# mp3guy/ElasticFusion

Measured on AMD Instinct MI355X. Metric: frames/s per GPU, 640x480 3-level ICP+fuse, higher is better.
Workload: dtype f32

## Files before the change

elasticfusion_amd/build.py:

```python
from __future__ import annotations

import os
import subprocess
import sys

HERE = os.path.dirname(os.path.abspath(__file__))
CSRC = os.path.join(HERE, "csrc")
LIB = os.path.join(HERE, "libefusion_hip.so")
FAST_LIB = os.path.join(HERE, "libefusion_hip_fast.so")
NOFMA_LIB = LIB
VARIANTS = {
    "fast": ["-DEF_FAST_BUILD"],
    "reforder": ["-DEF_FAST_BUILD", "-DEF_REF_ORDER"],
    "nofma_fast": ["-DEF_FORCE_FAST_ORDER"],
    "clocks": ["-DEF_STAGE_CLOCKS"],
    "fast_clocks": ["-DEF_FAST_BUILD", "-DEF_STAGE_CLOCKS"],
    "ldlt_wave": ["-DEF_LDLT_WAVE"],
    "ldlt_wave_clocks": ["-DEF_LDLT_WAVE", "-DEF_STAGE_CLOCKS"],
    "nopairs": ["-DEF_NO_VISIT_PAIRS"],
    "nopairs_clocks": ["-DEF_NO_VISIT_PAIRS", "-DEF_STAGE_CLOCKS"],
    "p_icp": ["-DEF_RT_WITH_PAIRS_ICP"],
    "p_search": ["-DEF_RT_WITH_PAIRS_SEARCH"],
    "p_rgb": ["-DEF_RT_WITH_PAIRS_RGB"],
    "p_all": ["-DEF_RT_WITH_PAIRS_ICP", "-DEF_RT_WITH_PAIRS_SEARCH", "-DEF_RT_WITH_PAIRS_RGB"],
    "shfl": ["-DEF_RT_SHFL_REDUCE"],
    "sepsc": ["-DEF_SEPARATE_SIN_COS"],
    "pyrstages": ["-DEF_PYR_STAGES"],
    "deep": ["-DEF_DEEP_PIPE"],
    "sepinputs": ["-DEF_SEPARATE_INPUTS"],
    "sepmerge": ["-DEF_SEPARATE_MERGE"],
    "pre_vpair": ["-DEF_PRE_VPAIR"],
    "prep_late": ["-DEF_RT_PREPARE_LATE"],
    "p_nostream": ["-DEF_RT_NO_PAIRS_STREAM"],
    "sepscan": ["-DEF_SEPARATE_SCAN"],
    "endwave": ["-DEF_END_ONE_WAVE"],
    "pre_pertap": ["-DEF_PRE_SCALE_PER_TAP"],
    "assoc_late": ["-DEF_ASSOC_LATE_LOADS"],
    "resolveall": ["-DEF_RESOLVE_ALL_MAPS"],
    "splat_early": ["-DEF_SPLAT_EARLY_LOADS"],
    "resolvetally": ["-DEF_RESOLVE_TALLY"],
    "modeone": ["-DEF_FT_MODE_ONE"],
    "modeone_clocks": ["-DEF_FT_MODE_ONE", "-DEF_STAGE_CLOCKS"],
    "norepl": ["-DEF_FT_REPL=1", "-DEF_FT_REPL_A=1"],
    "norepl_clocks": ["-DEF_FT_REPL=1", "-DEF_FT_REPL_A=1", "-DEF_STAGE_CLOCKS"],
    "lanesweep": ["-DEF_FT_LANE_SWEEP"],
    "lanesweep_clocks": ["-DEF_FT_LANE_SWEEP", "-DEF_STAGE_CLOCKS"],
    "pipepoll": ["-DEF_FT_PIPELINED_POLL"],
    "pipepoll_clocks": ["-DEF_FT_PIPELINED_POLL", "-DEF_STAGE_CLOCKS"],
    "alltaps": ["-DEF_CLEAN_ALL_TAPS"],
    "r6m": ["-DEF_SEPARATE_SCAN", "-DEF_END_ONE_WAVE"],
}
SHIM_LIB = os.path.join(HERE, "libefusion.so")
SOURCES = ["ef_track_kernels.hip", "ef_map_kernels.hip", "ef_context.hip", "ef_ferns.hip"]
FLAGS = ["--offload-arch=gfx950", "-O3", "-std=c++17", "-fPIC", "-ffp-contract=off", "-fno-fast-math",
         "-Wall", "-Wno-unused-function", "-Wno-unused-result"]


def _hipcc() -> str:
    for c in (os.environ.get("HIPCC"), "/opt/rocm/bin/hipcc", "hipcc"):
        if c and (os.path.isabs(c) and os.path.exists(c) or not os.path.isabs(c)):
            return c
    raise RuntimeError("hipcc not found")


def needs_build() -> bool:
    if not os.path.exists(LIB) or not os.path.exists(SHIM_LIB):
        return True
    t = os.path.getmtime(LIB)
    root = os.path.dirname(HERE)
    deps = [os.path.join(CSRC, f) for f in os.listdir(CSRC) if f.endswith((".hip", ".inc", ".hpp", ".h"))]
    deps += [os.path.join(root, "include", "ef_hip.h"), os.path.join(root, "include", "ElasticFusion.h"), os.path.join(root, "include", "efusion_klg.hpp"), os.path.join(root, "include", "efusion_jpeg.hpp"),
             os.path.join(root, "tools", "efusion_replay.cpp"), __file__]
    replay = os.path.join(HERE, "efusion_replay")
    return not os.path.exists(replay) or any(os.path.getmtime(d) > min(t, os.path.getmtime(replay)) for d in deps)


def build(force: bool = False, verbose: bool = False) -> str:
    if not force and not needs_build():
        return LIB
    objs = []
    procs = []
    for src in SOURCES:
        obj = os.path.join(CSRC, src.replace(".hip", ".o"))
        cmd = [_hipcc(), *FLAGS, *os.environ.get("EF_HIPCC_FLAGS", "").split(), "-c", os.path.join(CSRC, src), "-o", obj]
        if verbose:
            print(" ".join(cmd), flush=True)
        procs.append((src, subprocess.Popen(cmd, stdout=subprocess.PIPE, stderr=subprocess.STDOUT, text=True)))
        objs.append(obj)
    for src, p in procs:
        out, _ = p.communicate()
        if p.returncode != 0:
            raise RuntimeError(f"hipcc failed on {src}:\n{out}")
        if verbose and out.strip():
            print(out)
    cmd = [_hipcc(), "--offload-arch=gfx950", "-shared", "-fPIC", "-o", LIB, *objs, "-Wl,-rpath,/opt/rocm/lib"]
    r = subprocess.run(cmd, stdout=subprocess.PIPE, stderr=subprocess.STDOUT, text=True)
    if r.returncode != 0:
        raise RuntimeError(f"link failed:\n{r.stdout}")
    cmd = [_hipcc(), "--offload-arch=gfx950", "-O2", "-std=c++17", "-fPIC", "-ffp-contract=off", "-shared", "-o", SHIM_LIB,
           os.path.join(CSRC, "efusion_shim.hip"), "-L" + HERE, "-lefusion_hip", "-lz", "-ldl", "-Wl,-rpath,$ORIGIN", "-Wl,-rpath,/opt/rocm/lib"]
    r = subprocess.run(cmd, stdout=subprocess.PIPE, stderr=subprocess.STDOUT, text=True)
    if r.returncode != 0:
        raise RuntimeError(f"libefusion.so build failed:\n{r.stdout}")
    replay = os.path.join(HERE, "efusion_replay")
    cmd = ["g++", "-O2", "-std=c++17", os.path.join(os.path.dirname(HERE), "tools", "efusion_replay.cpp"), "-o", replay, "-L" + HERE,
           "-lefusion", "-lefusion_hip", "-lz", "-ldl", "-Wl,-rpath,$ORIGIN", "-Wl,-rpath,/opt/rocm/lib", "-Wl,-rpath-link," + HERE]
    r = subprocess.run(cmd, stdout=subprocess.PIPE, stderr=subprocess.STDOUT, text=True)
    if r.returncode != 0:
        raise RuntimeError(f"efusion_replay build failed:\n{r.stdout}")
    return LIB


def build_variant(name: str, extra_flags: list[str]) -> str:
    extra_flags = VARIANTS.get(name, []) + list(extra_flags)
    target = os.path.join(HERE, f"libefusion_hip_{name}.so")
    objs = []
    procs = []
    for src in SOURCES:
        obj = os.path.join(CSRC, src.replace(".hip", f"_{name}.o"))
        procs.append((src, subprocess.Popen([_hipcc(), *FLAGS, *extra_flags, "-c", os.path.join(CSRC, src), "-o", obj], stdout=subprocess.PIPE,
                                            stderr=subprocess.STDOUT, text=True)))
        objs.append(obj)
    for src, p in procs:
        out, _ = p.communicate()
        if p.returncode != 0:
            raise RuntimeError(f"hipcc failed on {src}:\n{out}")
    r = subprocess.run([_hipcc(), "--offload-arch=gfx950", "-shared", "-fPIC", "-o", target, *objs, "-Wl,-rpath,/opt/rocm/lib"], stdout=subprocess.PIPE,
                       stderr=subprocess.STDOUT, text=True)
    if r.returncode != 0:
        raise RuntimeError(f"link failed:\n{r.stdout}")
    return target


if __name__ == "__main__":
    if "--variant" in sys.argv:
        i = sys.argv.index("--variant")
        print(build_variant(sys.argv[i + 1], sys.argv[i + 2:]))
    else:
        print(build(force="--force" in sys.argv, verbose=True))
```

elasticfusion_amd/csrc/ef_context.hip:

```cpp
#include <hip/hip_runtime.h>
#include <math.h>
#include <cmath>
#include <stdio.h>
#include <string.h>
#include <limits>
#include <string>
#include <thread>
#include <vector>

#include "../../include/ef_hip.h"
#include "ef_linalg_dev.hpp"
#include "ef_solve_dev.hpp"
#include "ef_map.hpp"
#include "ef_deform_solver.hpp"
#include "ef_track.hpp"

namespace {

thread_local std::string g_create_error;

struct StageTimer {
  const char* name;
  hipEvent_t a, b;
  bool used;
};

}

struct ef_ctx {
  ef_config cfg;
  hipStream_t stream = nullptr;
  bool own_stream = false;
  std::string err;
  efm::Cam cam;
  eft::Intr intr;
  const float maxDepthProcessed = 20.0f;
  uint8_t* rgb = nullptr;
  uint16_t* depth_raw = nullptr;
  uint16_t* depth_filtered = nullptr;
  float* depth_metric = nullptr;
  float* depth_metric_filtered = nullptr;
  uint8_t* rgb_alt = nullptr;
  uint16_t* depth_raw_alt = nullptr;
  uint16_t* depth_filtered_alt = nullptr;
  float* depth_metric_alt = nullptr;
  float* depth_metric_filtered_alt = nullptr;
  hipStream_t in_stream = nullptr;
  hipEvent_t ev_input_done = nullptr, ev_track_done = nullptr, ev_staged = nullptr;
  hipEvent_t ev_frame_done[2] = {nullptr, nullptr};
  int frame_parity = 0;
  int overlap_mode = 1;
  bool overlap = false;
  bool events_live = false;
  static constexpr int RING = 3;
  uint8_t* h_rgb_ring[RING] = {};
  uint16_t* h_depth_ring[RING] = {};
  uint8_t* d_rgb_ring[RING] = {};
  uint16_t* d_depth_ring[RING] = {};
  hipEvent_t ev_h2d[RING] = {};
  hipStream_t copy_stream = nullptr;
  unsigned host_seq = 0;
  unsigned mark_value = 0;
  unsigned* h_consumed = nullptr;
  unsigned* d_consumed = nullptr;
  unsigned* h_abort = nullptr;
  unsigned* d_abort = nullptr;
  eft::Pyramid pyr{};
  eft::TrackState* st = nullptr;
  efm::IndexMaps im{};
  efm::PredictMaps pm{};
  efm::FillMaps fm{};
  unsigned long long* zbuf = nullptr;
  efm::SurfelSoA maps[2]{};
  int cur = 0;
  efm::SurfelSoA shadow{};
  bool reference_download = false;
  uint32_t capacity = 0;
  uint32_t* winner = nullptr;
  efm::Candidates cand{};
  efm::CompactScratch cs{};
  int* overflow = nullptr;
  double* traj = nullptr;
  int traj_cap = 0;
  std::vector<int64_t> stamps;
  int tick = 1;
  std::vector<void*> allocs;
  bool tally_by_consumer = false;
  bool tally_pending = false;
  bool timing = false;
  std::vector<StageTimer> timers;
  float* graph_dev = nullptr;
  int graph_nodes = 0, graph_is_fern = 0;
  float* synth_depth = nullptr;
  float* rays = nullptr;
  int icp_count_thresh = 35000;
  float icp_err_thresh = 5e-05f, cov_thresh = 1e-05f;
  int deforms = 0;
  const float* bil_table = nullptr;
  eft::Pyramid pyr2{};
  eft::TrackState* st2 = nullptr;
  efm::PredictMaps old{};
  float* cons_dev = nullptr;
  float* h_cons = nullptr;
  eft::TrackState* h_states = nullptr;
  ef_loop_solver solver = nullptr;
  void* solver_user = nullptr;
  bool builtin_solver = false;
  int64_t last_deform_time = 0;
  float* nodes_dev = nullptr;
  std::vector<float> h_nodes;
  ef_local_loop loop{};
  std::vector<double> loop_constraints;
  std::vector<float> loop_graph;
  ef_closure* closure = nullptr;
  ef_global_loop gloop{};
  std::string fern_tracker_error;
  int fern_w = 0, fern_h = 0;
  uchar4* view_img_dev = nullptr;
  float4* view_vert_dev = nullptr;
  float4* view_norm_dev = nullptr;
  uint8_t* h_view = nullptr;
  eft::Pyramid pyr3{};
  eft::TrackState* st3 = nullptr;
  eft::Intr intr3{};
  float4* fern_maps_dev = nullptr;
  float* h_nodes_pinned = nullptr;
  int* fern_table_dev = nullptr;
  int fern_num = 0, fern_table_version = -1;
  uint8_t* fern_codes_dev = nullptr;
  uint8_t* h_codes = nullptr;
  uint8_t* h_codes_end = nullptr;
  uint8_t* h_view_end = nullptr;
  hipEvent_t ev_end_record = nullptr;
  bool end_pending = false, end_lost = false;
  int end_tick = 0;
  int n_nodes_host = 0;
  double h_pose[16] = {1, 0, 0, 0, 0, 1, 0, 0, 0, 0, 1, 0, 0, 0, 0, 1};
  bool reloc = false, lost = false, last_frame_recovery = false, tracking_ok = true;
  int tracking_count = 0;
  eft::TrackState h_reloc{};
  bool use_graph = false;
  bool track_only = false;
  bool no_resident = false;
  bool fused_step = false;
  int persistent = 1;
  struct TrackGraph { hipGraphExec_t exec = nullptr; const void* key = nullptr; eft::TrackParams tp{}; eft::TrackTail tail{}; };
  TrackGraph tgraph[2];
  int ktime_every = 0;
  std::vector<hipEvent_t> kt_start, kt_stop;
  eft::KernelProbe probe{nullptr, nullptr, 0, 0};
  std::vector<hipEvent_t> ks_start, ks_stop;
  eft::KernelProbe probe_splat{nullptr, nullptr, 0, 0};
  std::vector<hipEvent_t> ka_start, ka_stop;
  eft::KernelProbe probe_all{nullptr, nullptr, 0, 0};
  hipStream_t debug_stream = nullptr;
  unsigned long long* render_zbuf = nullptr;
  size_t render_zbuf_n = 0;
  uint8_t* render_out = nullptr;
  size_t render_out_bytes = 0;
  bool ids_on = false, ids_bad = false;
  unsigned* ids_state = nullptr;
  int label_C = 0, label_cur = 0;
  float* label_tab[2] = {};
  uint32_t* label_ids[2] = {};
  size_t label_rows = 0, label_bound = 0;
  size_t label_known = 0, label_known_frames = 0, label_ev_frames = 0;
  unsigned* label_count_h = nullptr;
  hipEvent_t label_ev = nullptr;
  bool label_ev_pending = false;
  uint32_t* label_index = nullptr;
  size_t label_index_n = 0;
  uint8_t* label_stage = nullptr;
  size_t label_stage_bytes = 0;
  uint64_t map_gen = 1, query_gen = 0;
  float query_cell = EF_QUERY_DEFAULT_CELL, query_built_cell = 0.f;
  int query_lanes = 0;
  float4* query_sorted = nullptr;
  uint32_t* query_rows = nullptr;
  size_t query_cap = 0;
  uint32_t* query_cells = nullptr;
  size_t query_cells_cap = 0;
  uint32_t query_nb = 0, query_n = 0;
  uint8_t* query_stage = nullptr;
  size_t query_stage_bytes = 0;
  uint8_t* reg_slabs = nullptr;
  size_t reg_slabs_bytes = 0;
  double* reg_sums_h = nullptr;
  uint8_t* reg_stage = nullptr;
  size_t reg_stage_bytes = 0;
};

namespace {

#define EF_HIP(ctx, expr)                                                                       \
  do {                                                                                          \
    hipError_t _e = (expr);                                                                     \
    if (_e != hipSuccess) {                                                                     \
      (ctx)->err = std::string(#expr) + ": " + hipGetErrorString(_e);                           \
      return EF_EHIP;                                                                           \
    }                                                                                           \
  } while (0)

struct DeviceGuard {
  int prev = -1;
  bool switched = false;
  explicit DeviceGuard(const ef_ctx* c) {
    if (c && hipGetDevice(&prev) == hipSuccess && prev != c->cfg.device) switched = hipSetDevice(c->cfg.device) == hipSuccess;
  }
  ~DeviceGuard() {
    if (switched) (void)hipSetDevice(prev);
  }
  DeviceGuard(const DeviceGuard&) = delete;
  DeviceGuard& operator=(const DeviceGuard&) = delete;
};

template <typename T>
int dev_alloc(ef_ctx* c, T** p, size_t n, int fill = 0) {
  void* q = nullptr;
  hipError_t e = hipMalloc(&q, n * sizeof(T));
  if (e != hipSuccess) {
    c->err = std::string("hipMalloc: ") + hipGetErrorString(e);
    return EF_ENOMEM;
  }
  e = hipMemsetAsync(q, fill, n * sizeof(T), c->stream);
  if (e != hipSuccess) {
// ... 459 lines not shown
  const uint8_t* rgb_in = fold_copies ? rgb_src : c->rgb;
#ifdef EF_SEPARATE_INPUTS
  const bool joint_inputs = false;
#else
  const bool joint_inputs = track_this && !overlap && !c->timing;
#endif
  if (!joint_inputs && !efm::preprocess_depth(depth_in, W, H, c->cfg.depth_cut, c->depth_filtered, c->depth_metric, c->depth_metric_filtered, sb, 0u,
                             track_this ? rgb_in : nullptr, c->pyr.nextImage[0], fold_copies ? c->rgb : nullptr, c->bil_table)) {
    c->err = "bilateral weight table missing on this device";
    return EF_EHIP;
  }
  timer_end(c, "Preprocess");
  if (overlap && overlap_mode == 2) EF_HIP(c, hipStreamWaitEvent(sb, c->ev_track_done, 0));
  if (track_this && overlap)
    eft::build_pyramids_frame_side(c->pyr, c->depth_filtered, c->intr, c->maxDepthProcessed, nullptr, sb, nullptr);
  if (overlap) EF_HIP(c, hipEventRecord(c->ev_input_done, sb));

  const bool rgbOnly = c->cfg.rgb_only != 0;
  if ((int)c->stamps.size() >= c->traj_cap) {
    const int r = grow_trajectory(c);
    if (r != EF_OK) return r;
  }
  const int log_slot = (int)c->stamps.size();
  c->stamps.push_back(timestamp);
  if (c->tick == 1) {
    if (overlap) EF_HIP(c, hipStreamWaitEvent(s, c->ev_input_done, 0));
    timer_begin(c, "feedbackBuffers");
    efm::seed_map(c->cam, c->rgb, c->depth_metric, c->depth_metric_filtered, c->tick, c->maxDepthProcessed, c->maps[c->cur],
                  &c->st->map_counts[c->cur], c->cs, s);
    eft::init_first_rgb(c->pyr, c->rgb, s);
    if (log_slot >= 0) eft::log_pose(c->st, c->traj, log_slot, s);
    if (want_events) EF_HIP(c, hipEventRecord(c->ev_track_done, s));
    timer_end(c, "feedbackBuffers");
  } else {
    if (!in_T_wc) {
      eft::TrackParams tp;
      tp.rgbOnly = rgbOnly;
      tp.pyramid = c->cfg.pyramid != 0;
      tp.fastOdom = c->cfg.fast_odom != 0;
      tp.so3 = c->cfg.so3 != 0;
      tp.icpWeight = c->cfg.icp_weight;
      tp.persistent = c->persistent;
      tp.fused_step = c->fused_step ? 1 : 0;
  tp.no_resident = c->no_resident ? 1 : 0;
      tp.distThres = 0.10f;
      tp.angleThres = sinf(20.f * 3.14159254f / 180.f);
      const bool rgb = tp.rgbOnly || tp.icpWeight < 100;
      timer_begin(c, "odomInit");
      const eft::FramePreprocess fp{depth_in, c->cfg.depth_cut, c->bil_table, c->depth_filtered, c->depth_metric, c->depth_metric_filtered, rgb_in,
                                    fold_copies ? c->rgb : nullptr};
      eft::init_icp_model(c->pyr, (const float*)c->pm.vertex, (const float*)c->pm.normal, (const float*)c->fm.vertex,
                          (const float*)c->fm.normal, c->st, 6.0f , s, (const uint8_t*)c->pm.image,
                          (const uint8_t*)c->fm.image, c->cfg.frame_to_frame_rgb != 0, joint_inputs ? &fp : nullptr, c->tally_pending);
      c->tally_pending = false;
      if (overlap) {
        eft::build_pyramids_model_side(c->pyr, nullptr, nullptr, false, c->st, s);
        EF_HIP(c, hipStreamWaitEvent(s, c->ev_input_done, 0));
      } else {
        eft::build_pyramids(c->pyr, c->depth_filtered, c->intr, c->maxDepthProcessed, nullptr, nullptr, false, nullptr, c->st, s, nullptr, rgb);
      }
      if (rgb && overlap) eft::init_rgb_sobel(c->pyr, s);
      timer_end(c, "odomInit");
      timer_begin(c, "odom");
      const bool sample = c->ktime_every > 0 && (c->tick % c->ktime_every) == 0;
      if (c->use_graph && !sample && !c->timing) tp.persistent = 0;
      eft::TrackTail tail{};
      if (c->use_graph && !sample && !c->timing) {
        const void* key = c->pyr.nextImage[0];
        ef_ctx::TrackGraph* g = nullptr;
        for (auto& cand : c->tgraph)
          if (cand.exec && cand.key == key && !memcmp(&cand.tp, &tp, sizeof(tp))) g = &cand;
        if (!g) {
          g = (c->tgraph[0].exec && c->tgraph[0].key != key) ? &c->tgraph[1] : &c->tgraph[0];
          if (g->exec) { (void)hipGraphExecDestroy(g->exec); g->exec = nullptr; }
          eft::track_prepare(c->pyr, tp, s);
          eft::Pyramid pyr_copy = c->pyr;
          hipGraph_t graph = nullptr;
          EF_HIP(c, hipStreamBeginCapture(s, hipStreamCaptureModeThreadLocal));
          g->tail = eft::track(pyr_copy, c->st, c->intr, tp, s, nullptr);
          hipError_t ce = hipStreamEndCapture(s, &graph);
          if (ce == hipSuccess) ce = hipGraphInstantiate(&g->exec, graph, nullptr, nullptr, 0);
          if (graph) (void)hipGraphDestroy(graph);
          if (ce != hipSuccess) {
            g->exec = nullptr;
            c->err = std::string("hipGraph capture of the tracker: ") + hipGetErrorString(ce);
            return EF_EHIP;
          }
          g->key = key;
          memcpy(&g->tp, &tp, sizeof(tp));
        }
        EF_HIP(c, hipGraphLaunch(g->exec, s));
        eft::track_swap(c->pyr, tp);
        tail = g->tail;
      } else {
        tail = eft::track(c->pyr, c->st, c->intr, tp, s, sample ? &c->probe : nullptr, sample && c->probe_all.start ? &c->probe_all : nullptr);
      }
      eft::track_end(c->st, tail, rgb, weightMultiplier, log_slot >= 0 ? c->traj : nullptr, log_slot, s, eft::tracker_abort_word(c->pyr), c->d_abort);
      timer_end(c, "odom");
      c->tracking_ok = true;
      if (c->reloc) {
        EF_HIP(c, hipMemcpyAsync(&c->h_reloc, c->st, sizeof(eft::TrackState), hipMemcpyDeviceToHost, s));
        EF_HIP(c, hipStreamSynchronize(s));
        c->tracking_ok = c->h_reloc.lastICPError < 1e-04;
        if (!c->lost) {
          if (!reloc_covariance_ok(c->h_reloc)) c->tracking_ok = false;
          if (!c->tracking_ok) {
            if (++c->tracking_count > 10) c->lost = true;
          } else {
            c->tracking_count = 0;
          }
        } else if (c->last_frame_recovery) {
          if (!reloc_covariance_ok(c->h_reloc)) c->tracking_ok = false;
          if (c->tracking_ok) {
            c->lost = false;
            c->tracking_count = 0;
          }
          c->last_frame_recovery = false;
        }
      }
    } else {
      c->tracking_ok = true;
      if (overlap) EF_HIP(c, hipStreamWaitEvent(s, c->ev_input_done, 0));
      eft::pose_injected(c->st, in_T_wc, true, weightMultiplier, true, log_slot >= 0 ? c->traj : nullptr, log_slot, s);
    }
    if (want_events) EF_HIP(c, hipEventRecord(c->ev_track_done, s));
    if (c->cfg.close_loops) {
      int fern_graph = 0;
      if (c->closure) {
        timer_begin(c, "globalLoop");
        do_predict(c, false);
        c->last_frame_recovery = false;
        const int r = global_loop_closure(c, log_slot, &fern_graph);
        timer_end(c, "globalLoop");
        if (r != EF_OK) return r;
      }
      if (c->lost) {
        memset(&c->loop, 0, sizeof(c->loop));
      } else if (!fern_graph) {
        timer_begin(c, "localLoop");
        const int r = local_loop_closure(c, log_slot, c->closure != nullptr);
        timer_end(c, "localLoop");
        if (r != EF_OK) return r;
      } else {
        memset(&c->loop, 0, sizeof(c->loop));
      }
    }
    if (!rgbOnly && c->tracking_ok && !c->lost && !c->track_only) {
      timer_begin(c, "indexMap");
      const bool sample_splat = c->ktime_every > 0 && (c->tick % c->ktime_every) == 0 && c->probe_splat.start;
      efm::IndexMaps im_assoc = c->im;
#ifndef EF_RESOLVE_ALL_MAPS
      im_assoc.color_time = nullptr;
#endif
      efm::predict_indices(c->cam, c->st->T_cw, c->tick, c->maps[c->cur], &c->st->map_counts[c->cur], c->maxDepthProcessed, c->cfg.time_delta, c->zbuf,
                           im_assoc, s, sample_splat ? &c->probe_splat : nullptr);
      timer_end(c, "indexMap");
      timer_begin(c, "Fuse::Data+Update");
#ifdef EF_SEPARATE_MERGE
      const bool defer_merge = false;
#else
      const bool defer_merge = !c->timing;
#endif
      efm::fuse(c->cam, c->st->pose_f, c->tick, c->rgb, c->depth_metric, c->depth_metric_filtered, c->im, c->maxDepthProcessed,
                &c->st->weighting, c->maps[c->cur], &c->st->map_counts[c->cur], c->cand, c->winner, s, defer_merge);
      if (c->reference_download && !defer_merge) efm::copy_map(c->maps[c->cur], &c->st->map_counts[c->cur], c->shadow, s);
      timer_end(c, "Fuse::Data+Update");
      timer_begin(c, "indexMap2");
      efm::predict_indices(c->cam, c->st->T_cw, c->tick, c->maps[c->cur], &c->st->map_counts[c->cur], c->maxDepthProcessed, c->cfg.time_delta, c->zbuf,
                           c->im, s, nullptr, defer_merge ? &c->cand : nullptr, c->winner);
      if (c->reference_download && defer_merge) efm::copy_map(c->maps[c->cur], &c->st->map_counts[c->cur], c->shadow, s);
      timer_end(c, "indexMap2");
      efm::Deformation def{c->graph_dev, c->graph_nodes, c->synth_depth, c->graph_is_fern, c->maxDepthProcessed};
      if (c->graph_nodes > 0 && !c->graph_is_fern)
        efm::synthesize_depth(c->cam, c->st->T_cw, c->maps[c->cur], &c->st->map_counts[c->cur], c->maxDepthProcessed, c->cfg.confidence, c->tick,
                              c->tick - c->cfg.time_delta, 65535, c->zbuf, c->synth_depth, s, c->rays);
      timer_begin(c, "Fuse::Copy");
      c->cs.flip ^= 1;
      efm::clean(c->cam, c->st->T_cw, c->tick, c->im, c->cfg.confidence, c->cfg.time_delta, c->maps[c->cur], &c->st->map_counts[c->cur], c->cand,
                 c->winner, c->maps[c->cur ^ 1], &c->st->map_counts[c->cur ^ 1], c->capacity, c->cs, c->overflow, s,
                 c->graph_nodes > 0 ? &def : nullptr);
      c->graph_nodes = 0;
      c->cur ^= 1;
      timer_end(c, "Fuse::Copy");
    } else {
      c->graph_nodes = 0;
    }
  }
  timer_begin(c, "IndexMap::ACTIVE");
  do_predict(c);
  timer_end(c, "IndexMap::ACTIVE");
  if (c->closure) {
    timer_begin(c, "ferns");
    int r = flush_end_record(c);
    if (r == EF_OK) r = enqueue_end_record(c);
    timer_end(c, "ferns");
    if (r != EF_OK) return r;
  }
  if (want_events && c->overlap_mode == 2) EF_HIP(c, hipEventRecord(c->ev_frame_done[c->frame_parity], s));
  c->events_live = want_events;
  if (!c->lost) c->tick++;
  EF_HIP(c, hipGetLastError());
  return EF_OK;
}

int ctx_init(ef_ctx* c) {
  const ef_config& g = c->cfg;
  const int W = g.width, H = g.height;
  const size_t P = (size_t)W * H;
  hipStream_t s = c->stream;
  EF_ALLOC(c, c->rgb, P * 3);
  EF_ALLOC(c, c->depth_raw, P);
  EF_ALLOC(c, c->depth_filtered, P);
  EF_ALLOC(c, c->depth_metric, P);
  EF_ALLOC(c, c->depth_metric_filtered, P);
  EF_ALLOC(c, c->rgb_alt, P * 3);
  EF_ALLOC(c, c->depth_raw_alt, P);
  EF_ALLOC(c, c->depth_filtered_alt, P);
  EF_ALLOC(c, c->depth_metric_alt, P);
  EF_ALLOC(c, c->depth_metric_filtered_alt, P);
  EF_HIP(c, hipStreamCreateWithFlags(&c->in_stream, hipStreamNonBlocking));
  for (auto& e : c->ev_frame_done) EF_HIP(c, hipEventCreateWithFlags(&e, hipEventDisableTiming));
  EF_HIP(c, hipEventCreateWithFlags(&c->ev_input_done, hipEventDisableTiming));
  EF_HIP(c, hipEventCreateWithFlags(&c->ev_track_done, hipEventDisableTiming));
  EF_HIP(c, hipEventCreateWithFlags(&c->ev_staged, hipEventDisableTiming));
  EF_HIP(c, hipStreamCreateWithFlags(&c->copy_stream, hipStreamNonBlocking));
  for (int i = 0; i < ef_ctx::RING; ++i) {
    EF_HIP(c, hipEventCreateWithFlags(&c->ev_h2d[i], hipEventDisableTiming));
    EF_HIP(c, hipHostMalloc((void**)&c->h_rgb_ring[i], P * 3));
    EF_HIP(c, hipHostMalloc((void**)&c->h_depth_ring[i], P * 2));
    EF_ALLOC(c, c->d_rgb_ring[i], P * 3);
    EF_ALLOC(c, c->d_depth_ring[i], P);
  }
  EF_HIP(c, hipHostMalloc((void**)&c->h_consumed, sizeof(unsigned), hipHostMallocMapped));
  *c->h_consumed = 0u;
  EF_HIP(c, hipHostGetDevicePointer((void**)&c->d_consumed, c->h_consumed, 0));
  EF_HIP(c, hipHostMalloc((void**)&c->h_abort, 4 * sizeof(unsigned), hipHostMallocMapped));
  memset(c->h_abort, 0, 4 * sizeof(unsigned));
  EF_HIP(c, hipHostGetDevicePointer((void**)&c->d_abort, c->h_abort, 0));
  c->pyr.width = W;
  c->pyr.height = H;
  for (int i = 0; i < eft::NUM_PYRS; ++i) {
    const size_t n = (size_t)(W >> i) * (H >> i);
    EF_ALLOC(c, c->pyr.depth_tmp[i], n);
    EF_ALLOC(c, c->pyr.vmap_curr[i], 3 * n);
    EF_ALLOC(c, c->pyr.nmap_curr[i], 3 * n);
    EF_ALLOC(c, c->pyr.vmap_g_prev[i], 3 * n);
    EF_ALLOC(c, c->pyr.nmap_g_prev[i], 3 * n);
    EF_ALLOC(c, c->pyr.lastDepth[i], n);
    c->pyr.nextDepth[i] = c->pyr.lastDepth[i];
    EF_ALLOC(c, c->pyr.lastImage[i], n);
    EF_ALLOC(c, c->pyr.nextImage[i], n);
    EF_ALLOC(c, c->pyr.lastNextImage[i], n);
    EF_ALLOC(c, c->pyr.dIdx[i], n);
    EF_ALLOC(c, c->pyr.dIdy[i], n);
    EF_ALLOC(c, c->pyr.corres[i], n);
    EF_ALLOC(c, c->pyr.rgbMask[i], n);
  }
  EF_ALLOC(c, c->pyr.partials, (size_t)eft::PARTIAL_ALLOC_FLOATS);
  EF_ALLOC(c, c->st, 1);
  EF_ALLOC(c, c->im.index, P);
  EF_ALLOC(c, c->im.vert_conf, P);
  EF_ALLOC(c, c->im.color_time, P);
  EF_ALLOC(c, c->im.norm_rad, P);
  c->im.colmajor = 1;
  EF_ALLOC(c, c->pm.image, P);
  EF_ALLOC(c, c->pm.vertex, P);
  EF_ALLOC(c, c->pm.normal, P);
  EF_ALLOC(c, c->pm.time, P);
  EF_ALLOC(c, c->fm.image, P);
  EF_ALLOC(c, c->fm.vertex, P);
  EF_ALLOC(c, c->fm.normal, P);
  EF_ALLOC(c, c->zbuf, P, 0xFF);
  EF_ALLOC(c, c->graph_dev, 1024 * 16);
  EF_ALLOC(c, c->synth_depth, P);
  EF_ALLOC(c, c->rays, P * 4);
  EF_ALLOC(c, c->overflow, 1);
  c->capacity = g.max_surfels;
  for (int k = 0; k < 2; ++k) {
    EF_ALLOC(c, c->maps[k].pos_conf, c->capacity);
    EF_ALLOC(c, c->maps[k].col_time, c->capacity);
    EF_ALLOC(c, c->maps[k].nrm_rad, c->capacity);
  }
  EF_ALLOC(c, c->winner, c->capacity, 0xFF);
  c->cand.n = (W / 2) * (H / 2);
  EF_ALLOC(c, c->cand.pos_conf, c->cand.n);
  EF_ALLOC(c, c->cand.col_time, c->cand.n);
  EF_ALLOC(c, c->cand.nrm_rad, c->cand.n);
  EF_ALLOC(c, c->cand.best, c->cand.n);
  c->cs.max_chunks = (int)((c->capacity + (size_t)c->cand.n + 2 * P) / efm::CLEAN_ROW + 8);
  EF_ALLOC(c, c->cs.flags, (size_t)c->capacity + c->cand.n + 2 * P);
  EF_ALLOC(c, c->cs.chunk_count, c->cs.max_chunks);
  EF_ALLOC(c, c->cs.chunk_offset, c->cs.max_chunks);
  EF_ALLOC(c, c->cs.totals, 8);
  c->cs.max_groups = c->cs.max_chunks / efm::CLEAN_GROUP + 2;
  EF_ALLOC(c, c->cs.group_sum, 2 * (size_t)c->cs.max_groups * efm::CLEAN_GSTRIDE);
  if (g.close_loops) {
    c->pyr2.width = W;
    c->pyr2.height = H;
    for (int i = 0; i < eft::NUM_PYRS; ++i) {
      const size_t n = (size_t)(W >> i) * (H >> i);
      EF_ALLOC(c, c->pyr2.depth_tmp[i], n);
      EF_ALLOC(c, c->pyr2.vmap_curr[i], 3 * n);
      EF_ALLOC(c, c->pyr2.nmap_curr[i], 3 * n);
      EF_ALLOC(c, c->pyr2.vmap_g_prev[i], 3 * n);
      EF_ALLOC(c, c->pyr2.nmap_g_prev[i], 3 * n);
      EF_ALLOC(c, c->pyr2.lastDepth[i], n);
      EF_ALLOC(c, c->pyr2.nextDepth[i], n);
      EF_ALLOC(c, c->pyr2.lastImage[i], n);
      EF_ALLOC(c, c->pyr2.nextImage[i], n);
      EF_ALLOC(c, c->pyr2.lastNextImage[i], n);
      EF_ALLOC(c, c->pyr2.dIdx[i], n);
      EF_ALLOC(c, c->pyr2.dIdy[i], n);
      EF_ALLOC(c, c->pyr2.corres[i], n);
      EF_ALLOC(c, c->pyr2.rgbMask[i], n);
    }
    EF_ALLOC(c, c->pyr2.partials, (size_t)eft::PARTIAL_ALLOC_FLOATS);
    EF_ALLOC(c, c->st2, 1);
    EF_ALLOC(c, c->old.image, P);
    EF_ALLOC(c, c->old.vertex, P);
    EF_ALLOC(c, c->old.normal, P);
    EF_ALLOC(c, c->old.time, P);
    EF_ALLOC(c, c->cons_dev, (size_t)(W / 20) * (H / 20) * 4 + 4);
    EF_ALLOC(c, c->nodes_dev, (size_t)1024 * 4 + 4);
    EF_HIP(c, hipHostMalloc((void**)&c->h_cons, ((size_t)(W / 20) * (H / 20) * 4 + 4) * sizeof(float)));
    EF_HIP(c, hipHostMalloc((void**)&c->h_states, 3 * sizeof(eft::TrackState)));
    hipLaunchKernelGGL(k_init_state, dim3(1), dim3(64), 0, s, c->st2, (W / 20) * (H / 20), W * H);
  }
  c->traj_cap = 1 << 10;
  EF_ALLOC(c, c->traj, (size_t)c->traj_cap * 16);
  hipLaunchKernelGGL(k_init_state, dim3(1), dim3(64), 0, s, c->st, (W / 20) * (H / 20), W * H);
#ifndef EF_RESOLVE_TALLY
  c->tally_by_consumer = (W / 20) * (H / 20) <= 1024;
#endif
  efm::build_ray_table(c->cam, c->rays, s);
  const double I16[16] = {1, 0, 0, 0, 0, 1, 0, 0, 0, 0, 1, 0, 0, 0, 0, 1};
  eft::pose_injected(c->st, I16, false, 1.0f, false, nullptr, 0, s);
  eft::pose_injected(c->st, I16, true, 1.0f, false, nullptr, 0, s);
  EF_HIP(c, hipStreamSynchronize(s));
  return EF_OK;
}

void ctx_free(ef_ctx* c) {
  if (c->in_stream) (void)hipStreamSynchronize(c->in_stream);
  if (c->stream) (void)hipStreamSynchronize(c->stream);
  if (c->stream) eft::persistent_chain_forget(c->stream);
  if (c->in_stream) (void)hipStreamDestroy(c->in_stream);
  for (hipEvent_t e : {c->ev_input_done, c->ev_track_done, c->ev_staged, c->ev_frame_done[0], c->ev_frame_done[1]})
    if (e) (void)hipEventDestroy(e);
  for (void* p : c->allocs) (void)hipFree(p);
  if (c->h_abort) (void)hipHostFree(c->h_abort);
  if (c->copy_stream) { (void)hipStreamSynchronize(c->copy_stream); (void)hipStreamDestroy(c->copy_stream); }
  for (int i = 0; i < ef_ctx::RING; ++i) {
    if (c->ev_h2d[i]) (void)hipEventDestroy(c->ev_h2d[i]);
    if (c->h_rgb_ring[i]) (void)hipHostFree(c->h_rgb_ring[i]);
    if (c->h_depth_ring[i]) (void)hipHostFree(c->h_depth_ring[i]);
  }
  if (c->h_consumed) (void)hipHostFree(c->h_consumed);
  if (c->h_cons) (void)hipHostFree(c->h_cons);
  if (c->h_states) (void)hipHostFree(c->h_states);
  if (c->h_view) (void)hipHostFree(c->h_view);
  if (c->h_view_end) (void)hipHostFree(c->h_view_end);
  if (c->h_codes) (void)hipHostFree(c->h_codes);
  if (c->h_codes_end) (void)hipHostFree(c->h_codes_end);
  if (c->ev_end_record) (void)hipEventDestroy(c->ev_end_record);
  if (c->h_nodes_pinned) (void)hipHostFree(c->h_nodes_pinned);
  if (c->closure) ef_closure_destroy(c->closure);
  for (auto& t : c->timers) { (void)hipEventDestroy(t.a); (void)hipEventDestroy(t.b); }
  for (auto e : c->kt_start) (void)hipEventDestroy(e);
  for (auto e : c->kt_stop) (void)hipEventDestroy(e);
  for (auto& g : c->tgraph)
    if (g.exec) (void)hipGraphExecDestroy(g.exec);
  if (c->debug_stream) { (void)hipStreamSynchronize(c->debug_stream); (void)hipStreamDestroy(c->debug_stream); }
  for (auto e : c->ka_start) (void)hipEventDestroy(e);
  for (auto e : c->ka_stop) (void)hipEventDestroy(e);
  for (auto e : c->ks_start) (void)hipEventDestroy(e);
  for (auto e : c->ks_stop) (void)hipEventDestroy(e);
  if (c->render_zbuf) (void)hipFree(c->render_zbuf);
  if (c->render_out) (void)hipFree(c->render_out);
  for (int k = 0; k < 2; ++k) {
    if (c->label_tab[k]) (void)hipFree(c->label_tab[k]);
    if (c->label_ids[k]) (void)hipFree(c->label_ids[k]);
  }
  if (c->ids_state) (void)hipFree(c->ids_state);
  if (c->label_index) (void)hipFree(c->label_index);
  if (c->label_stage) (void)hipFree(c->label_stage);
  if (c->label_count_h) (void)hipHostFree(c->label_count_h);
  if (c->label_ev) (void)hipEventDestroy(c->label_ev);
  if (c->query_sorted) (void)hipFree(c->query_sorted);
  if (c->query_rows) (void)hipFree(c->query_rows);
  if (c->query_cells) (void)hipFree(c->query_cells);
  if (c->query_stage) (void)hipFree(c->query_stage);
  if (c->reg_slabs) (void)hipFree(c->reg_slabs);
  if (c->reg_sums_h) (void)hipHostFree(c->reg_sums_h);
  if (c->reg_stage) (void)hipFree(c->reg_stage);
  if (c->own_stream && c->stream) (void)hipStreamDestroy(c->stream);
}

int ids_prepare(ef_ctx* c, const char* fn);
int ids_uploaded(ef_ctx* c, uint32_t count);

}

extern "C" {

void ef_default_config(ef_config* cfg) {
  memset(cfg, 0, sizeof(*cfg));
  cfg->width = 640; cfg->height = 480;
  cfg->fx = 528; cfg->fy = 528; cfg->cx = 320; cfg->cy = 240;
  cfg->time_delta = 2147483647 / 2;
  cfg->confidence = 10.0f;
  cfg->depth_cut = 3.0f;
  cfg->icp_weight = 10.0f;
  cfg->fast_odom = 0; cfg->so3 = 1; cfg->frame_to_frame_rgb = 0; cfg->pyramid = 1; cfg->rgb_only = 0;
  cfg->close_loops = 0;
  cfg->max_surfels = 4u * 1024u * 1024u;
  cfg->device = 0;
  cfg->stream = nullptr;
}

int ef_create(const ef_config* cfg, ef_ctx** out) {
  if (!cfg || !out) { g_create_error = "null argument"; return EF_EINVAL; }
  if (cfg->width <= 0 || cfg->height <= 0 || (cfg->width % 4) || (cfg->height % 4) || cfg->fx <= 0 || cfg->fy <= 0) {
    g_create_error = "width/height must be positive multiples of 4 and focal lengths positive";
    return EF_EINVAL;
  }
// ... 477 lines not shown
  if (r != EF_OK) return r;
  if (n > max_surfels) n = max_surfels;
  *count = n;
  if (!surfels || !n) return EF_OK;
  float* tmp = nullptr;
  EF_HIP(c, hipMalloc((void**)&tmp, (size_t)n * 48));
  efm::soa_to_aos(c->reference_download ? c->shadow : c->maps[c->cur], n, tmp, c->stream);
  hipError_t e = hipMemcpyAsync(surfels, tmp, (size_t)n * 48, hipMemcpyDeviceToHost, c->stream);
  if (e == hipSuccess) e = hipStreamSynchronize(c->stream);
  (void)hipFree(tmp);
  EF_HIP(c, e);
  return EF_OK;
}
int ef_set_reference_download(ef_ctx* c, int on) {
  if (!c) return EF_EINVAL;
  DeviceGuard dg_(c);
  if (on && !c->shadow.pos_conf) {
    EF_ALLOC(c, c->shadow.pos_conf, c->capacity);
    EF_ALLOC(c, c->shadow.col_time, c->capacity);
    EF_ALLOC(c, c->shadow.nrm_rad, c->capacity);
  }
  c->reference_download = on != 0;
  return EF_OK;
}
int ef_map_upload(ef_ctx* c, const float* surfels, uint32_t count) {
  if (!c || (!surfels && count)) return EF_EINVAL;
  DeviceGuard dg_(c);
  if (count > c->capacity) { c->err = "ef_map_upload: count exceeds max_surfels"; return EF_ECAPACITY; }
  ++c->map_gen;
  float* tmp = nullptr;
  if (count) {
    EF_HIP(c, hipMalloc((void**)&tmp, (size_t)count * 48));
    hipError_t e = hipMemcpyAsync(tmp, surfels, (size_t)count * 48, hipMemcpyHostToDevice, c->stream);
    if (e == hipSuccess) {
      efm::aos_to_soa(tmp, count, c->maps[c->cur], c->stream);
      e = hipStreamSynchronize(c->stream);
    }
    (void)hipFree(tmp);
    EF_HIP(c, e);
  }
  hipLaunchKernelGGL(k_set_count, dim3(1), dim3(64), 0, c->stream, &c->st->map_counts[c->cur], count);
  if (c->ids_on) return ids_uploaded(c, count);
  return EF_OK;
}
int ef_get_pose_qt(ef_ctx* c, double* q4_t3) {
  if (!c || !q4_t3) return EF_EINVAL;
  DeviceGuard dg_(c);
  eft::TrackState h;
  EF_HIP(c, hipMemcpyAsync(&h, c->st, sizeof(h), hipMemcpyDeviceToHost, c->stream));
  EF_HIP(c, hipStreamSynchronize(c->stream));
  for (int i = 0; i < 4; ++i) q4_t3[i] = h.q[i];
  for (int i = 0; i < 3; ++i) q4_t3[4 + i] = h.t[i];
  return EF_OK;
}
int ef_restore_state(ef_ctx* c, int tick, const double* q4_t3, const uint8_t* rgb_prev, const uint16_t* depth_prev) {
  if (!c || !q4_t3 || !rgb_prev || !depth_prev || tick < 2) return EF_EINVAL;
  DeviceGuard dg_(c);
  ++c->map_gen;
  hipStream_t s = c->stream;
  const int W = c->cam.cols, H = c->cam.rows;
  if (c->closure) {
    const int fr = flush_end_record(c);
    if (fr != EF_OK) return fr;
  }
  EF_HIP(c, hipMemcpyAsync(c->rgb, rgb_prev, (size_t)W * H * 3, hipMemcpyHostToDevice, s));
  EF_HIP(c, hipMemcpyAsync(c->depth_raw, depth_prev, (size_t)W * H * 2, hipMemcpyHostToDevice, s));
  EF_HIP(c, hipStreamSynchronize(s));
  if (!efm::preprocess_depth(c->depth_raw, W, H, c->cfg.depth_cut, c->depth_filtered, c->depth_metric, c->depth_metric_filtered, s, 0u, nullptr,
                             nullptr, nullptr, c->bil_table)) {
    c->err = "bilateral weight table missing on this device";
    return EF_EHIP;
  }
  eft::init_first_rgb(c->pyr, c->rgb, s);
  efl::SE3 T;
  for (int i = 0; i < 4; ++i) T.q[i] = q4_t3[i];
  for (int i = 0; i < 3; ++i) T.t[i] = q4_t3[4 + i];
  eft::pose_restored(c->st, T.q, T.t, s);
  c->tick = tick;
  c->lost = c->last_frame_recovery = false;
  c->tracking_ok = true;
  c->tracking_count = 0;
  c->graph_nodes = 0;
  const int r = do_predict(c);
  EF_HIP(c, hipGetLastError());
  return r;
}
int ef_write_freiburg(const char* path, const double* T_wc16_array, const int64_t* timestamps, int n) {
  if (!path || (n > 0 && (!T_wc16_array || !timestamps))) return EF_EINVAL;
  FILE* f = fopen(path, "w");
  if (!f) return EF_EINVAL;
  for (int i = 0; i < n; ++i) {
    const efl::SE3 S = efl::se3_from_matrix(T_wc16_array + (size_t)i * 16);
    fprintf(f, "%.6f %g %g %g %g %g %g %g\n", (double)timestamps[i] / 1000000.0, S.t[0], S.t[1], S.t[2], S.q[0], S.q[1], S.q[2], S.q[3]);
  }
  fclose(f);
  return EF_OK;
}
int ef_write_ply(const char* path, const float* surfels, uint32_t count, float confidence_threshold) {
  if (!path || (count > 0 && !surfels)) return EF_EINVAL;
  uint32_t valid = 0;
  for (uint32_t i = 0; i < count; ++i) valid += surfels[(size_t)i * 12 + 3] > confidence_threshold;
  FILE* f = fopen(path, "wb");
  if (!f) return EF_EINVAL;
  fprintf(f, "ply\nformat binary_little_endian 1.0\nelement vertex %u\nproperty float x\nproperty float y\nproperty float z\n"
             "property uchar red\nproperty uchar green\nproperty uchar blue\nproperty float nx\nproperty float ny\nproperty float nz\n"
             "property float radius\nend_header\n", valid);
  for (uint32_t i = 0; i < count; ++i) {
    const float* s = surfels + (size_t)i * 12;
    if (!(s[3] > confidence_threshold)) continue;
    const int col = (int)s[4];
    const unsigned char rgbc[3] = {(unsigned char)((col >> 16) & 0xFF), (unsigned char)((col >> 8) & 0xFF), (unsigned char)(col & 0xFF)};
    const float nr[4] = {s[8] * -1, s[9] * -1, s[10] * -1, s[11]};
    fwrite(s, sizeof(float), 3, f);
    fwrite(rgbc, 1, 3, f);
    fwrite(nr, sizeof(float), 4, f);
  }
  fclose(f);
  return EF_OK;
}
int ef_save_freiburg(ef_ctx* c, const char* path) {
  if (!c || !path) return EF_EINVAL;
  DeviceGuard dg_(c);
  const int n = (int)c->stamps.size();
  std::vector<double> T((size_t)n * 16);
  int got = 0;
  int r = ef_get_trajectory(c, T.data(), nullptr, n, &got);
  if (r != EF_OK) return r;
  r = ef_write_freiburg(path, T.data(), c->stamps.data(), got);
  if (r != EF_OK) c->err = std::string("cannot open ") + path;
  return r;
}
int ef_save_ply(ef_ctx* c, const char* path) {
  if (!c || !path) return EF_EINVAL;
  DeviceGuard dg_(c);
  uint32_t n = 0;
  int r = ef_map_count(c, &n);
  if (r != EF_OK) return r;
  std::vector<float> m((size_t)n * 12);
  r = ef_map_download(c, m.data(), n, &n);
  if (r != EF_OK) return r;
  r = ef_write_ply(path, m.data(), n, c->cfg.confidence);
  if (r != EF_OK) c->err = std::string("cannot open ") + path;
  return r;
}
int ef_set_rgb_only(ef_ctx* c, int v) { if (!c) return EF_EINVAL; c->cfg.rgb_only = v; return EF_OK; }
int ef_set_icp_weight(ef_ctx* c, float v) { if (!c) return EF_EINVAL; c->cfg.icp_weight = v; return EF_OK; }
int ef_set_pyramid(ef_ctx* c, int v) { if (!c) return EF_EINVAL; c->cfg.pyramid = v; return EF_OK; }
int ef_set_fast_odom(ef_ctx* c, int v) { if (!c) return EF_EINVAL; c->cfg.fast_odom = v; return EF_OK; }
int ef_set_so3(ef_ctx* c, int v) { if (!c) return EF_EINVAL; c->cfg.so3 = v; return EF_OK; }
int ef_set_frame_to_frame_rgb(ef_ctx* c, int v) { if (!c) return EF_EINVAL; c->cfg.frame_to_frame_rgb = v; return EF_OK; }
int ef_set_confidence_threshold(ef_ctx* c, float v) { if (!c) return EF_EINVAL; c->cfg.confidence = v; return EF_OK; }
int ef_set_depth_cutoff(ef_ctx* c, float v) { if (!c) return EF_EINVAL; c->cfg.depth_cut = v; return EF_OK; }

int ef_get_image(ef_ctx* c, int which, void* dst, size_t bytes) {
  if (!c || !dst) return EF_EINVAL;
  DeviceGuard dg_(c);
  const size_t P = (size_t)c->cam.cols * c->cam.rows;
  const void* src = nullptr;
  size_t need = 0;
  switch (which) {
    case EF_IMG_DEPTH_FILTERED: src = c->depth_filtered; need = P * 2; break;
    case EF_IMG_DEPTH_METRIC: src = c->depth_metric; need = P * 4; break;
    case EF_IMG_DEPTH_METRIC_FILTERED: src = c->depth_metric_filtered; need = P * 4; break;
    case EF_IMG_PREDICT_IMAGE: src = c->pm.image; need = P * 4; break;
    case EF_IMG_PREDICT_VERTEX: src = c->pm.vertex; need = P * 16; break;
    case EF_IMG_PREDICT_NORMAL: src = c->pm.normal; need = P * 16; break;
    case EF_IMG_PREDICT_TIME: src = c->pm.time; need = P * 2; break;
    case EF_IMG_FILL_IMAGE: src = c->fm.image; need = P * 4; break;
    case EF_IMG_FILL_VERTEX: src = c->fm.vertex; need = P * 16; break;
    case EF_IMG_FILL_NORMAL: src = c->fm.normal; need = P * 16; break;
    case EF_IMG_INDEX: src = c->im.index; need = P * 4; break;
    case EF_IMG_VERT_CONF: src = c->im.vert_conf; need = P * 16; break;
    case EF_IMG_COLOR_TIME: src = c->im.color_time; need = P * 16; break;
    case EF_IMG_NORM_RAD: src = c->im.norm_rad; need = P * 16; break;
    case EF_IMG_OLD_IMAGE: src = c->old.image; need = P * 4; break;
    case EF_IMG_OLD_VERTEX: src = c->old.vertex; need = P * 16; break;
    case EF_IMG_OLD_NORMAL: src = c->old.normal; need = P * 16; break;
    case EF_IMG_OLD_TIME: src = c->old.time; need = P * 2; break;
    default: c->err = "ef_get_image: unknown image"; return EF_EINVAL;
  }
  if (!src) { c->err = "ef_get_image: this image only exists in a close_loops context"; return EF_ESTATE; }
  if (bytes < need) { c->err = "ef_get_image: destination too small"; return EF_EINVAL; }
  void* tmp = nullptr;
  if (c->im.colmajor && which >= EF_IMG_INDEX && which <= EF_IMG_NORM_RAD) {
    EF_HIP(c, hipMalloc(&tmp, need));
    const int W = c->cam.cols, H = c->cam.rows;
    const dim3 g((unsigned)((P + 255) / 256));
    if (which == EF_IMG_INDEX) hipLaunchKernelGGL(k_to_rowmajor<uint32_t>, g, dim3(256), 0, c->stream, (const uint32_t*)src, W, H, (uint32_t*)tmp);
    else hipLaunchKernelGGL(k_to_rowmajor<float4>, g, dim3(256), 0, c->stream, (const float4*)src, W, H, (float4*)tmp);
    src = tmp;
  }
  hipError_t e = hipMemcpyAsync(dst, src, need, hipMemcpyDeviceToHost, c->stream);
  if (e == hipSuccess) e = hipStreamSynchronize(c->stream);
  if (tmp) (void)hipFree(tmp);
  EF_HIP(c, e);
  return EF_OK;
}
int ef_get_image_resized(ef_ctx* c, int which, int factor, void* dst, size_t bytes) {
  if (!c || !dst || factor < 1) return EF_EINVAL;
  DeviceGuard dg_(c);
  const int W = c->cam.cols, H = c->cam.rows, dw = W / factor, dh = H / factor;
  const void* src = nullptr;
  int elem = 0;
  switch (which) {
    case EF_IMG_PREDICT_IMAGE: src = c->pm.image; elem = 4; break;
    case EF_IMG_PREDICT_VERTEX: src = c->pm.vertex; elem = 16; break;
    case EF_IMG_PREDICT_NORMAL: src = c->pm.normal; elem = 16; break;
    case EF_IMG_PREDICT_TIME: src = c->pm.time; elem = 2; break;
    case EF_IMG_FILL_IMAGE: src = c->fm.image; elem = 4; break;
    case EF_IMG_FILL_VERTEX: src = c->fm.vertex; elem = 16; break;
    case EF_IMG_FILL_NORMAL: src = c->fm.normal; elem = 16; break;
    case EF_IMG_OLD_IMAGE: src = c->old.image; elem = 4; break;
    case EF_IMG_OLD_VERTEX: src = c->old.vertex; elem = 16; break;
    case EF_IMG_OLD_NORMAL: src = c->old.normal; elem = 16; break;
    case EF_IMG_OLD_TIME: src = c->old.time; elem = 2; break;
    default: c->err = "ef_get_image_resized: a predicted, fill-in or inactive-prediction image"; return EF_EINVAL;
  }
  if (!src) { c->err = "ef_get_image_resized: this image only exists in a close_loops context"; return EF_ESTATE; }
  const size_t need = (size_t)dw * dh * elem;
  if (dw == 0 || dh == 0 || bytes < need) { c->err = "ef_get_image_resized: destination too small"; return EF_EINVAL; }
  void* tmp = nullptr;
  EF_HIP(c, hipMalloc(&tmp, need));
  const dim3 g((unsigned)((dw * dh + 255) / 256));
  if (elem == 16) hipLaunchKernelGGL(k_resize_nearest<float4>, g, dim3(256), 0, c->stream, (const float4*)src, W, dw, dh, factor, (float4*)tmp);
  else if (elem == 4) hipLaunchKernelGGL(k_resize_nearest<uint32_t>, g, dim3(256), 0, c->stream, (const uint32_t*)src, W, dw, dh, factor, (uint32_t*)tmp);
  else hipLaunchKernelGGL(k_resize_nearest<uint16_t>, g, dim3(256), 0, c->stream, (const uint16_t*)src, W, dw, dh, factor, (uint16_t*)tmp);
  hipError_t e = hipMemcpyAsync(dst, tmp, need, hipMemcpyDeviceToHost, c->stream);
  if (e == hipSuccess) e = hipStreamSynchronize(c->stream);
  (void)hipFree(tmp);
  EF_HIP(c, e);
  return EF_OK;
}
int ef_get_tracker_buffer(ef_ctx* c, int which, int level, void* dst, size_t bytes) {
  if (!c || !dst || level < 0 || level >= eft::NUM_PYRS) return EF_EINVAL;
  DeviceGuard dg_(c);
  const size_t n = (size_t)(c->cam.cols >> level) * (c->cam.rows >> level);
  const void* src = nullptr;
  size_t need = 0;
  const eft::Pyramid& p = c->pyr;
  switch (which) {
    case 0: src = p.vmap_curr[level]; need = n * 12; break;
    case 1: src = p.nmap_curr[level]; need = n * 12; break;
    case 2: src = p.vmap_g_prev[level]; need = n * 12; break;
    case 3: src = p.nmap_g_prev[level]; need = n * 12; break;
    case 4: case 5: src = p.lastDepth[level]; need = n * 4; break;
    case 6: src = p.lastImage[level]; need = n; break;
    case 7: src = p.nextImage[level]; need = n; break;
    case 8: src = p.lastNextImage[level]; need = n; break;
    case 9: src = p.dIdx[level]; need = n * 2; break;
    case 10: src = p.dIdy[level]; need = n * 2; break;
    case 11: src = level == 0 ? c->depth_filtered : p.depth_tmp[level]; need = n * 2; break;
    default: c->err = "ef_get_tracker_buffer: unknown buffer"; return EF_EINVAL;
  }
  if (bytes < need) { c->err = "ef_get_tracker_buffer: destination too small"; return EF_EINVAL; }
  EF_HIP(c, hipMemcpyAsync(dst, src, need, hipMemcpyDeviceToHost, c->stream));
  EF_HIP(c, hipStreamSynchronize(c->stream));
  return EF_OK;
}

int ef_enable_timing(ef_ctx* c, int on) { if (!c) return EF_EINVAL; c->timing = on != 0; return EF_OK; }
int ef_get_timings(ef_ctx* c, ef_timing* out, int max, int* n) {
  if (!c || !n) return EF_EINVAL;
  DeviceGuard dg_(c);
  EF_HIP(c, hipStreamSynchronize(c->stream));
  int k = 0;
  for (auto& t : c->timers) {
    if (!t.used || k >= max) continue;
    float ms = 0.f;
    if (hipEventElapsedTime(&ms, t.a, t.b) != hipSuccess) ms = -1.f;
    if (out) { out[k].name = t.name; out[k].ms = ms; }
    ++k;
  }
  *n = k;
  return EF_OK;
}

int ef_kernel_timing(ef_ctx* c, int every_n_frames) {
  if (!c || every_n_frames < 0) return EF_EINVAL;
  DeviceGuard dg_(c);
  EF_HIP(c, hipStreamSynchronize(c->stream));
  c->ktime_every = every_n_frames;
  c->probe.used = 0;
  c->probe_splat.used = 0;
  c->probe_all.used = 0;
  if (every_n_frames > 0 && c->ka_start.empty()) {
    const int cap = 1024;
    c->ka_start.resize(cap);
    c->ka_stop.resize(cap);
    for (int i = 0; i < cap; ++i) {
      EF_HIP(c, hipEventCreate(&c->ka_start[i]));
      EF_HIP(c, hipEventCreate(&c->ka_stop[i]));
    }
    c->probe_all = eft::KernelProbe{c->ka_start.data(), c->ka_stop.data(), cap, 0};
  }
  if (every_n_frames > 0 && c->ks_start.empty()) {
    const int cap = 1024;
    c->ks_start.resize(cap);
    c->ks_stop.resize(cap);
    for (int i = 0; i < cap; ++i) {
      EF_HIP(c, hipEventCreate(&c->ks_start[i]));
      EF_HIP(c, hipEventCreate(&c->ks_stop[i]));
    }
    c->probe_splat = eft::KernelProbe{c->ks_start.data(), c->ks_stop.data(), cap, 0};
  }
  if (every_n_frames > 0 && c->kt_start.empty()) {
    const int cap = 4096;
    c->kt_start.resize(cap);
    c->kt_stop.resize(cap);
    for (int i = 0; i < cap; ++i) {
      EF_HIP(c, hipEventCreate(&c->kt_start[i]));
// ... 1430 lines not shown
```

elasticfusion_amd/csrc/ef_map.hpp:

```cpp
#pragma once
#include <hip/hip_runtime.h>
#include <stdint.h>
#include "ef_track.hpp"

namespace efm {

struct Cam { int cols, rows; float fx, fy, cx, cy; };

struct SurfelSoA {
  float4* pos_conf;
  float4* col_time;
  float4* nrm_rad;
};

constexpr unsigned long long ZBUF_EMPTY = 0xFFFFFFFFFFFFFFFFull;
constexpr unsigned WINNER_EMPTY = 0xFFFFFFFFu;
constexpr int CHUNK = 1024;
constexpr int CLEAN_ROW = 256;

struct IndexMaps {
  uint32_t* index;
  float4* vert_conf;
  float4* color_time;
  float4* norm_rad;
  int colmajor = 0;
};
__host__ __device__ inline int im_texel(const IndexMaps& im, const Cam& cam, int px, int py) {
  return im.colmajor ? px * cam.rows + py : py * cam.cols + px;
}
struct PredictMaps {
  uchar4* image;
  float4* vertex;
  float4* normal;
  uint16_t* time;
};
struct FillMaps {
  uchar4* image;
  float4* vertex;
  float4* normal;
};
struct Candidates {
  float4* pos_conf;
  float4* col_time;
  float4* nrm_rad;
  uint32_t* best;
  int n;
};
struct CompactScratch {
  uint8_t* flags;
  uint32_t* chunk_count;
  uint32_t* chunk_offset;
  uint32_t* totals;
  int max_chunks;
  uint32_t* group_sum = nullptr;
  int max_groups = 0;
  int flip = 0;
};
constexpr int CLEAN_GROUP = 32;
constexpr int CLEAN_GSTRIDE = 32;

const float* bilateral_table();
bool filter_depth(const uint16_t* raw, int cols, int rows, float maxD, uint16_t* filtered, hipStream_t s);
void metricise_depth(const uint16_t* in, int cols, int rows, float maxD, float* out, hipStream_t s);
bool preprocess_depth(const uint16_t* raw, int cols, int rows, float maxD, uint16_t* filtered, float* metric,
                      float* metric_filtered, hipStream_t s, unsigned extra_lds = 0, const uint8_t* rgb3 = nullptr, uint8_t* next0 = nullptr,
                      uint8_t* rgb_keep = nullptr, const float* table = nullptr);

void aos_to_soa(const float* aos, uint32_t count, SurfelSoA soa, hipStream_t s);
void soa_to_aos(SurfelSoA soa, uint32_t count, float* aos, hipStream_t s);
void copy_map(SurfelSoA src, const unsigned* count_dev, SurfelSoA dst, hipStream_t s);

void seed_map(const Cam& cam, const uint8_t* rgb3, const float* depth_metric, const float* depth_metric_filtered, int time,
              float maxDepth, SurfelSoA out, unsigned* count_dev, const CompactScratch& cs, hipStream_t s);

void predict_indices(const Cam& cam, const float* T_cw16_dev, int time, SurfelSoA map, const unsigned* count_dev, float maxDepth,
                     int timeDelta, unsigned long long* zbuf, IndexMaps out, hipStream_t s, eft::KernelProbe* probe = nullptr,
                     const struct Candidates* merge_cand = nullptr, const uint32_t* merge_winner = nullptr);
void combined_predict(const Cam& cam, const float* T_cw16_dev, SurfelSoA map, const unsigned* count_dev, float maxDepth,
                      float confThreshold, int time, int maxTime, int timeDelta, unsigned long long* zbuf, PredictMaps out,
                      FillMaps fill, const uint16_t* depth_filtered, const uint8_t* rgb3, bool passthroughImage,
                      unsigned* dense_counter, hipStream_t s,
                      unsigned* nonempty_flag = nullptr, unsigned nonempty_value = 0,
                      unsigned* consumed_mark = nullptr, unsigned consumed_value = 0,
                      const float* rays4 = nullptr);
void build_ray_table(const Cam& cam, float* rays4, hipStream_t s);
void synthesize_depth(const Cam& cam, const float* T_cw16_dev, SurfelSoA map, const unsigned* count_dev, float maxDepth,
                      float confThreshold, int time, int maxTime, int timeDelta, unsigned long long* zbuf, float* depth, hipStream_t s,
                      const float* rays4 = nullptr);
void fill_in(const Cam& cam, PredictMaps pred, const uint16_t* depth_filtered, const uint8_t* rgb3, bool passthrough,
             bool passthroughImage, FillMaps out, hipStream_t s);
void dense_count(const Cam& cam, const uchar4* image, unsigned* counter, hipStream_t s);

void fuse(const Cam& cam, const float* pose_f16_dev, int time, const uint8_t* rgb3, const float* depth_metric,
          const float* depth_metric_filtered, IndexMaps im, float maxDepth, const float* weighting_dev, SurfelSoA map,
          const unsigned* count_dev, Candidates cand, uint32_t* winner, hipStream_t s, bool defer_merge = false);
struct Deformation {
  const float* graph_dev;
  int nodes;
  const float* depth_dev;
  int is_fern;
  float max_depth;
};
void clean(const Cam& cam, const float* T_cw16_dev, int time, IndexMaps im, float confThreshold, int timeDelta, SurfelSoA map,
           const unsigned* count_dev, Candidates cand, uint32_t* winner, SurfelSoA out, unsigned* count_out_dev, uint32_t capacity,
           const CompactScratch& cs, int* overflow_flag, hipStream_t s, const Deformation* deform = nullptr);
void sample_graph(SurfelSoA map, const unsigned* count_dev, int stride, int max_nodes, float* out4, unsigned* n_out, hipStream_t s);
void candidates_to_aos(Candidates cand, float* aos, unsigned* count_dev, const CompactScratch& cs, hipStream_t s);

struct RenderArgs {
  Cam cam;
  float Tcw[16];
  float maxDepth, threshold;
  int drawUnstable, colorType, drawWindow, time, timeDelta;
};
struct RenderOut {
  uchar4* rgba;
  float* depth;
  float4* vertex;
  float4* normal;
  uint32_t* index;
};
void render_model(const RenderArgs& a, SurfelSoA map, const unsigned* count_dev, unsigned long long* zbuf, RenderOut out, hipStream_t s);

void ids_assign(SurfelSoA map, const unsigned* count_dev, unsigned* state, hipStream_t s);
void ids_check(SurfelSoA map, unsigned n, unsigned* flag, hipStream_t s);
void ids_zero(SurfelSoA map, const unsigned* count_dev, unsigned max_rows, hipStream_t s);
void ids_gather(SurfelSoA map, unsigned n, uint32_t* out, hipStream_t s);
struct LabelAlign {
  SurfelSoA map;
  const unsigned* count_dev;
  const uint32_t* ids_in;
  const float* tab_in;
  const unsigned* n_in;
  uint32_t* ids_out;
  float* tab_out;
  unsigned* n_out;
  int C;
  float prior;
};
struct LabelFuse {
  SurfelSoA map;
  const unsigned* count_dev;
  Cam cam;
  float Tcw[16];
  const uint32_t* index;
  const float* probs;
  float* tab;
  int C;
};
void labels_align(const LabelAlign& a, unsigned max_rows, hipStream_t s);
void labels_fuse(const LabelFuse& f, unsigned max_rows, hipStream_t s);
void labels_gather(const uint32_t* index, int P, const float* tab, int C, int32_t* label, float* prob, hipStream_t s);

struct QueryArgs {
  SurfelSoA map;
  const float4* sorted;
  const uint32_t* rows;
  const uint32_t* cells;
  unsigned mask;
  unsigned n_sorted;
  float inv_cell;
  const float* points;
  unsigned n;
  int k;
  float max_dist, r2, min_conf;
  uint32_t* row;
  float* dist2;
  uint32_t* id;
  float* plane;
  uint32_t* count;
};
constexpr int QUERY_MAX_RATIO = 16;
unsigned query_buckets(unsigned n);
void query_build(SurfelSoA map, unsigned n, float inv_cell, unsigned nb, uint32_t* cells, uint32_t* tile_sum, float4* sorted, uint32_t* rows,
                 hipStream_t s);
void query_run(const QueryArgs& a, int k, int lanes, hipStream_t s);

constexpr int REGISTER_SLOTS = 32;
constexpr int REGISTER_MAX_BLOCKS = 1536;
struct RegisterArgs {
  QueryArgs q;
  const float* normals;
  float R[9], t[3];
  float min_normal_cos;
  int gate;
  double* slabs;
  double* sums;
};
unsigned register_blocks(unsigned n);
void register_step(const RegisterArgs& a, hipStream_t s);

}
```

elasticfusion_amd/csrc/ef_map_kernels.hip:

```cpp
#include "ef_device.hpp"
#include <stdlib.h>
#include <mutex>
#include <hip/hip_ext.h>
#include "ef_map.hpp"

using namespace ef;

namespace efm {

namespace {

inline int ceil_div(int a, int b) { return (a + b - 1) / b; }
constexpr int SURFEL_GRID = 1024;
constexpr int BLK = 256;
constexpr int CLEAN_GRID = 4096;
static_assert(CLEAN_ROW == BLK, "clean kernels run one element per thread");
static_assert(CLEAN_GRID % 8 == 0, "xcd_row");

__device__ __forceinline__ uint32_t depth_key(float z) {
  const uint32_t b = __float_as_uint(z);
  return (b & 0x80000000u) ? ~b : (b | 0x80000000u);
}
__device__ __forceinline__ unsigned long long zkey(float z, uint32_t id) { return ((unsigned long long)depth_key(z) << 32) | id; }
__device__ __forceinline__ unsigned xcd_block() {
  const unsigned g = gridDim.x, x = blockIdx.x & 7u, slot = blockIdx.x >> 3;
  return x * (g >> 3) + (x < (g & 7u) ? x : (g & 7u)) + slot;
}
constexpr unsigned XCD_CHUNK = 32;
__device__ __forceinline__ bool xcd_row(unsigned nrows, unsigned it, unsigned& r) {
  const unsigned x = blockIdx.x & 7u, slot = blockIdx.x >> 3, per = gridDim.x >> 3;
  const unsigned local = slot + it * per;
  r = (x + 8u * (local / XCD_CHUNK)) * XCD_CHUNK + (local % XCD_CHUNK);
  return r < nrows;
}

__device__ __forceinline__ float pix_coord(int i, int n) {
  const float u = (float)((double)((float)i / (float)n) + 1.0 / (double)(2 * (float)n));
  return u * (float)n;
}
__device__ __forceinline__ float encodeColor(f3 c) {
  int rgb = (int)roundf(c.x * 255.0f);
  rgb = (rgb << 8) + (int)roundf(c.y * 255.0f);
  rgb = (rgb << 8) + (int)roundf(c.z * 255.0f);
  return (float)rgb;
}
__device__ __forceinline__ f3 decodeColor(float c) {
  const int ic = (int)c;
  return {(float)((ic >> 16) & 0xFF) / 255.0f, (float)((ic >> 8) & 0xFF) / 255.0f, (float)(ic & 0xFF) / 255.0f};
}
__device__ __forceinline__ float getRadius(float depth, float norm_z, float inv_fx, float inv_fy) {
  const float meanFocal = ((1.0f / fabsf(inv_fx)) + (1.0f / fabsf(inv_fy))) / 2.0f;
  const float sqrt2 = 1.41421356237f;
  const float radius = (depth / meanFocal) * sqrt2;
  const float radius_n = radius / fabsf(norm_z);
  return fminf(2.0f * radius, radius_n);
}
__device__ __forceinline__ float confidence(float x, float y, float cx, float cy, float weighting) {
  const float maxRadDist = 400, twoSigmaSquared = 0.72f;
  const float px = x - cx, py = y - cy;
  const float radialDist = sqrtf(px * px + py * py) / maxRadDist;
  return ef_expf(-(radialDist * radialDist) / twoSigmaSquared) * weighting;
}
struct DepthF {
  const float* d; int cols, rows;
  __device__ __forceinline__ float at(int x, int y) const { return d[clampi(y, 0, rows - 1) * cols + clampi(x, 0, cols - 1)]; }
};
__device__ __forceinline__ f3 getVertexF(const DepthF& D, int ix, int iy, float x, float y, float cx, float cy, float inv_fx, float inv_fy) {
  const float z = D.at(ix, iy);
  return {(x - cx) * z * inv_fx, (y - cy) * z * inv_fy, z};
}
__device__ __forceinline__ f3 half_sum(f3 a, f3 b) { return {(a.x + b.x) / 2, (a.y + b.y) / 2, (a.z + b.z) / 2}; }
__device__ __forceinline__ f3 getNormalF(const DepthF& D, f3 vPosition, int ix, int iy, float x, float y, float cx, float cy,
                                         float inv_fx, float inv_fy) {
  const f3 xf = getVertexF(D, ix + 1, iy, x + 1, y, cx, cy, inv_fx, inv_fy);
  const f3 xb = getVertexF(D, ix - 1, iy, x - 1, y, cx, cy, inv_fx, inv_fy);
  const f3 yf = getVertexF(D, ix, iy + 1, x, y + 1, cx, cy, inv_fx, inv_fy);
  const f3 yb = getVertexF(D, ix, iy - 1, x, y - 1, cx, cy, inv_fx, inv_fy);
  const f3 del_x = half_sum(xb, vPosition) - half_sum(xf, vPosition);
  const f3 del_y = half_sum(yb, vPosition) - half_sum(yf, vPosition);
  return normalized(cross(del_x, del_y));
}

__device__ __forceinline__ unsigned block_excl_scan(unsigned v, unsigned* lds, unsigned& total) {
  const int t = threadIdx.x, lane = t & 63, w = t >> 6;
  unsigned x = v;
#pragma unroll
  for (int off = 1; off < 64; off <<= 1) {
    const unsigned y = __shfl_up(x, off, 64);
    if (lane >= off) x += y;
  }
  __syncthreads();
  if (lane == 63) lds[w] = x;
  __syncthreads();
  unsigned base = 0, tot = 0;
#pragma unroll
  for (int i = 0; i < BLK / 64; ++i) {
    const unsigned s = lds[i];
    if (i < w) base += s;
    tot += s;
  }
  total = tot;
  return base + x - v;
}

__device__ __forceinline__ uint16_t bilateral_px(const uint16_t* __restrict__ raw, int cols, int rows, int x, int y, unsigned maxv) {
  const unsigned value = raw[y * cols + x];
  if (value > maxv || value < 300U) return 0;
  const float sigma_space2_inv_half = 0.024691358f, sigma_color2_inv_half = 0.000555556f;
  const int R = 6, D = R * 2 + 1;
  const int tx = min(x - D / 2 + D, cols), ty = min(y - D / 2 + D, rows);
  float sum1 = 0, sum2 = 0;
  for (int cy = max(y - D / 2, 0); cy < ty; ++cy)
    for (int cx = max(x - D / 2, 0); cx < tx; ++cx) {
      const unsigned tmp = raw[cy * cols + cx];
      const float space2 = ((float)x - (float)cx) * ((float)x - (float)cx) + ((float)y - (float)cy) * ((float)y - (float)cy);
      const float color2 = ((float)value - (float)tmp) * ((float)value - (float)tmp);
      const float weight = ef_expf(-(space2 * sigma_space2_inv_half + color2 * sigma_color2_inv_half));
      sum1 += (float)tmp * weight;
      sum2 += weight;
    }
  return (uint16_t)(unsigned)roundf(sum1 / sum2);
}
#include "ef_preprocess.inc"
__global__ void k_bilateral_table(float* __restrict__ table) {
  const int i = blockIdx.x * blockDim.x + threadIdx.x;
  if (i >= BIL_ROWS * BIL_COLS) return;
  const int r = i / BIL_COLS, k = i - r * BIL_COLS;
  const float sigma_space2_inv_half = 0.024691358f, sigma_color2_inv_half = 0.000555556f;
  const float space2 = (float)BIL.distinct[r];
  const float d = (float)k;
  const float color2 = d * d;
  table[i] = k < BIL_ZERO ? ef_expf(-(space2 * sigma_space2_inv_half + color2 * sigma_color2_inv_half)) : 0.0f;
}
template <bool WITH_METRIC>
__global__ void __launch_bounds__(256) k_preprocess(const uint16_t* __restrict__ raw, int cols, int rows, unsigned maxv, const float* __restrict__ table,
                                                     uint16_t* __restrict__ filtered, float* __restrict__ metric,
                                                     float* __restrict__ metric_filtered, const uint8_t* __restrict__ rgb3,
                                                     uint8_t* __restrict__ next0, uint8_t* __restrict__ rgb_keep) {
  preprocess_tile<WITH_METRIC>((int)blockIdx.x, (int)blockIdx.y, raw, cols, rows, maxv, table, filtered, metric, metric_filtered, rgb3, next0, rgb_keep);
}
__global__ void k_metricise(const uint16_t* __restrict__ in, int n, unsigned maxv, float* __restrict__ out) {
  const int i = blockIdx.x * blockDim.x + threadIdx.x;
  if (i < n) out[i] = metric_px(in[i], maxv);
}

__global__ void k_aos_to_soa(const float4* __restrict__ aos, uint32_t count, SurfelSoA soa) {
  const uint32_t i = blockIdx.x * blockDim.x + threadIdx.x;
  if (i >= count) return;
  soa.pos_conf[i] = aos[(size_t)i * 3];
  soa.col_time[i] = aos[(size_t)i * 3 + 1];
  soa.nrm_rad[i] = aos[(size_t)i * 3 + 2];
}
__global__ void k_soa_to_aos(SurfelSoA soa, uint32_t count, float4* __restrict__ aos) {
  const uint32_t i = blockIdx.x * blockDim.x + threadIdx.x;
  if (i >= count) return;
  aos[(size_t)i * 3] = soa.pos_conf[i];
  aos[(size_t)i * 3 + 1] = soa.col_time[i];
  aos[(size_t)i * 3 + 2] = soa.nrm_rad[i];
}

__device__ __forceinline__ unsigned dyn_n(const unsigned* count_dev, unsigned extra) { return (count_dev ? *count_dev : 0u) + extra; }

__global__ void __launch_bounds__(1024) k_scan_chunks(const uint32_t* __restrict__ counts, const unsigned* count_dev, unsigned extra,
                                                       uint32_t* __restrict__ offsets, uint32_t* total_out, unsigned* count_out = nullptr,
                                                       uint32_t capacity = 0, int* overflow_flag = nullptr, unsigned chunk = CHUNK) {
  __shared__ unsigned wsum[16];
  __shared__ unsigned carry_s;
  const unsigned n = dyn_n(count_dev, extra);
  const unsigned nchunks = (n + chunk - 1) / chunk;
  const int t = threadIdx.x, lane = t & 63, w = t >> 6;
  if (t == 0) carry_s = 0;
  __syncthreads();
  for (unsigned base = 0; base < nchunks; base += 1024) {
    const unsigned i = base + t;
    const unsigned v = i < nchunks ? counts[i] : 0u;
    unsigned x = v;
#pragma unroll
    for (int off = 1; off < 64; off <<= 1) {
      const unsigned y = __shfl_up(x, off, 64);
      if (lane >= off) x += y;
    }
    if (lane == 63) wsum[w] = x;
    __syncthreads();
    unsigned wb = 0, tot = 0;
    for (int k = 0; k < 16; ++k) {
      const unsigned s = wsum[k];
      if (k < w) wb += s;
      tot += s;
    }
    const unsigned carry = carry_s;
    if (i < nchunks) offsets[i] = carry + wb + x - v;
    __syncthreads();
    if (t == 0) carry_s = carry + tot;
    __syncthreads();
  }
  if (t == 0) {
    *total_out = carry_s;
    if (count_out) {
      unsigned tot = carry_s;
      if (tot > capacity) { tot = capacity; if (overflow_flag) *overflow_flag = 1; }
      *count_out = tot;
    }
  }
}

struct SeedArgs {
  Cam cam;
  const uint8_t* rgb3;
  const float* dm;
  const float* dmf;
  int time;
  float maxDepth;
};
__global__ void __launch_bounds__(BLK) k_seed_flags(const SeedArgs A, uint8_t* __restrict__ flags_raw, uint8_t* __restrict__ flags_filt,
                                                     uint32_t* __restrict__ cnt_raw, uint32_t* __restrict__ cnt_filt) {
  __shared__ unsigned lds[BLK / 64];
  const int P = A.cam.cols * A.cam.rows;
  const int c = blockIdx.x;
  unsigned nr = 0, nf = 0;
#pragma unroll
  for (int k = 0; k < 4; ++k) {
    const int e = c * CHUNK + threadIdx.x * 4 + k;
    if (e < P) {
      const int i = e / A.cam.rows, j = e - i * A.cam.rows;
      const float zr = A.dm[j * A.cam.cols + i], zf = A.dmf[j * A.cam.cols + i];
      const uint8_t fr = !(zr <= 0 || zr > A.maxDepth), ff = !(zf <= 0 || zf > A.maxDepth);
      flags_raw[e] = fr; flags_filt[e] = ff;
      nr += fr; nf += ff;
    }
  }
  unsigned tot;
  block_excl_scan(nr, lds, tot);
  if (threadIdx.x == 0) cnt_raw[c] = tot;
  block_excl_scan(nf, lds, tot);
  if (threadIdx.x == 0) cnt_filt[c] = tot;
}
__global__ void __launch_bounds__(BLK) k_seed_scatter(const SeedArgs A, const uint8_t* __restrict__ flags_raw,
                                                       const uint8_t* __restrict__ flags_filt, const uint32_t* __restrict__ off_raw,
                                                       const uint32_t* __restrict__ off_filt, const uint32_t* __restrict__ total_raw,
                                                       SurfelSoA out, unsigned* count_dev) {
  __shared__ unsigned lds[BLK / 64];
  const Cam cam = A.cam;
  const int P = cam.cols * cam.rows;
  const int c = blockIdx.x;
  const float inv_fx = 1.0f / cam.fx, inv_fy = 1.0f / cam.fy;
  uint8_t fr[4], ff[4];
  unsigned nr = 0, nf = 0;
#pragma unroll
  for (int k = 0; k < 4; ++k) {
    const int e = c * CHUNK + threadIdx.x * 4 + k;
    fr[k] = e < P ? flags_raw[e] : 0;
    ff[k] = e < P ? flags_filt[e] : 0;
    nr += fr[k]; nf += ff[k];
  }
  unsigned tot;
  unsigned pr = off_raw[c] + block_excl_scan(nr, lds, tot);
  unsigned pf = off_filt[c] + block_excl_scan(nf, lds, tot);
  const unsigned rawTotal = *total_raw;
  if (c == 0 && threadIdx.x == 0) *count_dev = rawTotal;
#pragma unroll
  for (int k = 0; k < 4; ++k) {
    const int e = c * CHUNK + threadIdx.x * 4 + k;
    if (e >= P) break;
    if (!fr[k] && !ff[k]) continue;
    const int i = e / cam.rows, j = e - i * cam.rows;
    const float x = pix_coord(i, cam.cols), y = pix_coord(j, cam.rows);
    if (fr[k]) {
      const DepthF D{A.dm, cam.cols, cam.rows};
      const f3 v = getVertexF(D, i, j, x, y, cam.cx, cam.cy, inv_fx, inv_fy);
      const uint8_t* cc = A.rgb3 + (size_t)(j * cam.cols + i) * 3;
      const f3 col{(float)cc[0] / 255.0f, (float)cc[1] / 255.0f, (float)cc[2] / 255.0f};
      out.pos_conf[pr] = make_float4(v.x, v.y, v.z, confidence(x, y, cam.cx, cam.cy, 1.0f));
      out.col_time[pr] = make_float4(encodeColor(col), 0.f, 1.f, (float)A.time);
      ++pr;
    }
    if (ff[k]) {
      const DepthF D{A.dmf, cam.cols, cam.rows};
      const f3 v = getVertexF(D, i, j, x, y, cam.cx, cam.cy, inv_fx, inv_fy);
      const f3 n = getNormalF(D, v, i, j, x, y, cam.cx, cam.cy, inv_fx, inv_fy);
      if (pf < rawTotal) out.nrm_rad[pf] = make_float4(n.x, n.y, n.z, getRadius(v.z, n.z, inv_fx, inv_fy));
      ++pf;
    }
  }
}

__device__ __forceinline__ void merge_surfel(const Candidates& cand, int r, uint32_t id, const SurfelSoA& map, int time, float4& s, float4& sc);
template <bool MERGE>
__global__ void __launch_bounds__(BLK) k_index_splat(const Cam cam, const float* __restrict__ T16, int time, SurfelSoA map,
                                                      const unsigned* __restrict__ count_dev, float maxDepth, int timeDelta,
                                                      unsigned long long* zbuf, int colmajor, Candidates cand, const uint32_t* __restrict__ winner) {
  const rt34 T = rt34_load16(T16);
  const unsigned count = *count_dev;
  const float ftime = (float)time, ftd = (float)timeDelta;
  for (unsigned id = blockIdx.x * blockDim.x + threadIdx.x; id < count; id += gridDim.x * blockDim.x) {
    float4 pc = map.pos_conf[id];
    float4 ct = map.col_time[id];
    if (MERGE) {
      const uint32_t r = winner[id];
      if (r != WINNER_EMPTY) merge_surfel(cand, (int)r, id, map, time, pc, ct);
    }
    const f3 p = xform(T, f3{pc.x, pc.y, pc.z});
    if (p.z > maxDepth || p.z < 0 || ftime - ct.w > ftd) continue;
    const float u = ((cam.fx * p.x) / p.z) + cam.cx;
    const float v = ((cam.fy * p.y) / p.z) + cam.cy;
    const float xn = (u - (float)cam.cols * 0.5f) / ((float)cam.cols * 0.5f), yn = (v - (float)cam.rows * 0.5f) / ((float)cam.rows * 0.5f);
    const double xw = ((double)xn + 1.0) * 0.5 * (double)cam.cols, yw = ((double)yn + 1.0) * 0.5 * (double)cam.rows;
    if (!(xw >= 0 && xw < cam.cols && yw >= 0 && yw < cam.rows)) continue;
    const int px = (int)floor(xw), py = (int)floor(yw);
    atomicMin(&zbuf[colmajor ? px * cam.rows + py : py * cam.cols + px], zkey(p.z, id));
  }
}
__global__ void __launch_bounds__(BLK) k_index_resolve(const Cam cam, const float* __restrict__ T16, SurfelSoA map,
                                                        unsigned long long* zbuf, IndexMaps out) {
  const int pi = blockIdx.x * blockDim.x + threadIdx.x;
  if (pi >= cam.cols * cam.rows) return;
  const unsigned long long key = zbuf[pi];
  if (key == ZBUF_EMPTY) {
    out.index[pi] = 0u;
    out.vert_conf[pi] = make_float4(0, 0, 0, 0);
    if (out.color_time) out.color_time[pi] = make_float4(0, 0, 0, 0);
    out.norm_rad[pi] = make_float4(0, 0, 0, 0);
    return;
  }
  zbuf[pi] = ZBUF_EMPTY;
  const uint32_t id = (uint32_t)key;
  const rt34 T = rt34_load16(T16);
  const float4 pc = map.pos_conf[id];
  const float4 nr = map.nrm_rad[id];
  const f3 p = xform(T, f3{pc.x, pc.y, pc.z});
  const f3 n = normalized(mul(T.R, f3{nr.x, nr.y, nr.z}));
  out.index[pi] = id;
  out.vert_conf[pi] = make_float4(p.x, p.y, p.z, pc.w);
  if (out.color_time) out.color_time[pi] = map.col_time[id];
  out.norm_rad[pi] = make_float4(n.x, n.y, n.z, nr.w);
}

struct Sprite {
  f3 p, n;
  float rad, conf;
  float u, v, hs;
  bool ok;
};
__device__ __forceinline__ Sprite make_sprite(const Cam& cam, const rt34& T, float4 pc, float4 ct, float4 nr, float maxDepth,
                                              float confThreshold, float ftime, float fmaxTime, float ftd) {
  Sprite S;
  S.ok = false;
  S.p = xform(T, f3{pc.x, pc.y, pc.z});
  if (S.p.z > maxDepth || S.p.z < 0 || pc.w < confThreshold || ftime - ct.w > ftd || ct.w > fmaxTime) return S;
  S.n = normalized(mul(T.R, f3{nr.x, nr.y, nr.z}));
  S.rad = nr.w;
  S.conf = pc.w;
  const f3 t1 = normalized(f3{S.n.y - S.n.z, -S.n.x, S.n.x});
  const f3 x1{(t1.x * S.rad) * 1.41421356f, (t1.y * S.rad) * 1.41421356f, (t1.z * S.rad) * 1.41421356f};
  const f3 y1 = cross(S.n, x1);
  const float fx = cam.fx, fy = cam.fy, cx = cam.cx, cy = cam.cy;
  const f3 a = S.p + x1, b = S.p + y1, c = S.p - y1, d = S.p - x1;
  const float q1x = ((fx * a.x) / a.z) + cx, q1y = ((fy * a.y) / a.z) + cy;
  const float q2x = ((fx * b.x) / b.z) + cx, q2y = ((fy * b.y) / b.z) + cy;
  const float q3x = ((fx * c.x) / c.z) + cx, q3y = ((fy * c.y) / c.z) + cy;
  const float q4x = ((fx * d.x) / d.z) + cx, q4y = ((fy * d.y) / d.z) + cy;
  const float xmin = fminf(q1x, fminf(q2x, fminf(q3x, q4x))), xmax = fmaxf(q1x, fmaxf(q2x, fmaxf(q3x, q4x)));
  const float ymin = fminf(q1y, fminf(q2y, fminf(q3y, q4y))), ymax = fmaxf(q1y, fmaxf(q2y, fmaxf(q3y, q4y)));
  if (q1x != q1x || q2x != q2x || q3x != q3x || q4x != q4x || q1y != q1y || q2y != q2y || q3y != q3y || q4y != q4y) return S;
  float size = fmaxf(0.f, fmaxf(fabsf(xmax - xmin), fabsf(ymax - ymin)));
  if (size != size) return S;
  size = fminf(fmaxf(size, 1.0f), 2047.0f);
  S.u = ((fx * S.p.x) / S.p.z) + cx;
  S.v = ((fy * S.p.y) / S.p.z) + cy;
  if (!(S.u >= 0 && S.u < (float)cam.cols && S.v >= 0 && S.v < (float)cam.rows)) return S;
  S.hs = size * 0.5f;
  S.ok = true;
  return S;
}
__device__ __forceinline__ f3 pixel_ray(const Cam& cam, int px, int py) {
  const float fcx = (float)px + 0.5f, fcy = (float)py + 0.5f;
  return normalized(f3{(fcx - cam.cx) / cam.fx, (fcy - cam.cy) / cam.fy, 1.0f});
}
__device__ __forceinline__ bool sprite_fragment_ray(const f3& Sp, const f3& Sn, float rad, float psn, const f3& l, float& z) {
  const float k = psn / dot(l, Sn);
  const f3 cp{k * l.x, k * l.y, k * l.z};
  const f3 diff = cp - Sp;
  if (!(dot(diff, diff) <= rad * rad)) return false;
  z = cp.z;
  return true;
}
__device__ __forceinline__ bool sprite_fragment(const Cam& cam, const Sprite& S, int px, int py, float& z) {
  return sprite_fragment_ray(S.p, S.n, S.rad, dot(S.p, S.n), pixel_ray(cam, px, py), z);
}
__global__ void k_ray_table(const Cam cam, float4* __restrict__ rays) {
  const int i = blockIdx.x * blockDim.x + threadIdx.x;
  if (i >= cam.cols * cam.rows) return;
  const int px = i / cam.rows, py = i - px * cam.rows;
  const f3 l = pixel_ray(cam, px, py);
  rays[i] = make_float4(l.x, l.y, l.z, 0.f);
}
#ifndef EF_SPLAT_LANES
#define EF_SPLAT_LANES 4
#endif
constexpr int SPLAT_LANES = EF_SPLAT_LANES;
#ifndef EF_SPLAT_TILED
constexpr int SPLAT_GRID = SURFEL_GRID * SPLAT_LANES;
#else
constexpr int SPLAT_ROUNDS = 2, SPLAT_CHUNK = SPLAT_ROUNDS * (BLK / SPLAT_LANES), SPLAT_TILE = 4096;
constexpr int SPLAT_GRID = 4096;
#endif
template <bool LUT>
__global__ void __launch_bounds__(BLK) k_surface_splat(const Cam cam, const float* __restrict__ T16, SurfelSoA map,
                                                        const unsigned* __restrict__ count_dev, float maxDepth, float confThreshold,
                                                        int time, int maxTime, int timeDelta, unsigned long long* zbuf,
                                                        unsigned* consumed_mark, unsigned consumed_value, const float4* __restrict__ rays) {
  if (consumed_mark && blockIdx.x == 0 && threadIdx.x == 0)
    __hip_atomic_store(consumed_mark, consumed_value, __ATOMIC_RELAXED, __HIP_MEMORY_SCOPE_SYSTEM);
  const rt34 T = rt34_load16(T16);
  const unsigned count = *count_dev;
  const unsigned sub = threadIdx.x % SPLAT_LANES;
#ifndef EF_SPLAT_TILED
  const unsigned stride = gridDim.x * blockDim.x / SPLAT_LANES;
  for (unsigned id = (blockIdx.x * blockDim.x + threadIdx.x) / SPLAT_LANES; id < count; id += stride) {
    const float4 pc = map.pos_conf[id];
#ifdef EF_SPLAT_EARLY_LOADS
    const float4 ct = map.col_time[id];
    const float4 nr = map.nrm_rad[id];
    if (pc.w < confThreshold) continue;
#else
    if (pc.w < confThreshold) continue;
    const float4 ct = map.col_time[id];
    const float4 nr = map.nrm_rad[id];
#endif
    const Sprite S = make_sprite(cam, T, pc, ct, nr, maxDepth, confThreshold, (float)time, (float)maxTime, (float)timeDelta);
    if (!S.ok) continue;
    const int px0 = max(0, (int)ceilf(S.u - S.hs - 0.5f)), px1 = min(cam.cols - 1, (int)ceilf(S.u + S.hs - 0.5f) - 1);
    const int py0 = max(0, (int)ceilf(S.v - S.hs - 0.5f)), py1 = min(cam.rows - 1, (int)ceilf(S.v + S.hs - 0.5f) - 1);
    const int hgt = py1 - py0 + 1, nfrag = (px1 - px0 + 1) * hgt;
    const float psn = dot(S.p, S.n);
    for (int f = (int)sub; f < nfrag; f += SPLAT_LANES) {
      const int fx = f / hgt, py = py0 + (f - fx * hgt), px = px0 + fx;
      const int zi = px * cam.rows + py;
      f3 l;
      if (LUT) { const float4 r = rays[zi]; l = f3{r.x, r.y, r.z}; }
      else l = pixel_ray(cam, px, py);
      float z;
      if (!sprite_fragment_ray(S.p, S.n, S.rad, psn, l, z)) continue;
      if (z != z) continue;
      unsigned long long* cell = &zbuf[zi];
      const unsigned long long key = zkey(z, id);
#if defined(EF_SPLAT_EARLYZ) && EF_SPLAT_EARLYZ == 1
      if (*(volatile unsigned long long*)cell <= key) continue;
#elif defined(EF_SPLAT_EARLYZ) && EF_SPLAT_EARLYZ == 2
      if (__hip_atomic_load(cell, __ATOMIC_RELAXED, __HIP_MEMORY_SCOPE_AGENT) <= key) continue;
#endif
      atomicMin(cell, key);
    }
  }
#else
  (void)rays;
  __shared__ unsigned long long tile[SPLAT_TILE];
  __shared__ int box[4];
  const unsigned group = threadIdx.x / SPLAT_LANES;
  for (unsigned c0 = blockIdx.x * SPLAT_CHUNK; c0 < count; c0 += gridDim.x * SPLAT_CHUNK) {
    if (threadIdx.x == 0) { box[0] = box[1] = 0x7fffffff; box[2] = box[3] = -1; }
    __syncthreads();
    Sprite S[SPLAT_ROUNDS];
    int px0[SPLAT_ROUNDS], px1[SPLAT_ROUNDS], py0[SPLAT_ROUNDS], py1[SPLAT_ROUNDS];
#pragma unroll
    for (int r = 0; r < SPLAT_ROUNDS; ++r) {
      const unsigned id = c0 + r * (BLK / SPLAT_LANES) + group;
      S[r].ok = false;
      px0[r] = py0[r] = 0;
      px1[r] = py1[r] = -1;
      if (id < count) {
        const float4 pc = map.pos_conf[id];
        if (!(pc.w < confThreshold)) {
          const float4 ct = map.col_time[id];
          const float4 nr = map.nrm_rad[id];
          S[r] = make_sprite(cam, T, pc, ct, nr, maxDepth, confThreshold, (float)time, (float)maxTime, (float)timeDelta);
        }
      }
      if (S[r].ok) {
        px0[r] = max(0, (int)ceilf(S[r].u - S[r].hs - 0.5f)); px1[r] = min(cam.cols - 1, (int)ceilf(S[r].u + S[r].hs - 0.5f) - 1);
        py0[r] = max(0, (int)ceilf(S[r].v - S[r].hs - 0.5f)); py1[r] = min(cam.rows - 1, (int)ceilf(S[r].v + S[r].hs - 0.5f) - 1);
        if (sub == 0 && px1[r] >= px0[r] && py1[r] >= py0[r]) {
          atomicMin(&box[0], px0[r]); atomicMin(&box[1], py0[r]);
          atomicMax(&box[2], px1[r]); atomicMax(&box[3], py1[r]);
        }
      }
    }
    __syncthreads();
    const int bx0 = box[0], by0 = box[1];
    const int bw = box[2] - bx0 + 1;
    const int th = bw > 0 ? min(box[3] - by0 + 1, SPLAT_TILE / bw) : 0;
    const int tn = bw > 0 ? bw * th : 0;
    for (int i = threadIdx.x; i < tn; i += BLK) tile[i] = ~0ull;
    __syncthreads();
#pragma unroll
    for (int r = 0; r < SPLAT_ROUNDS; ++r) {
      if (!S[r].ok) continue;
      const unsigned id = c0 + r * (BLK / SPLAT_LANES) + group;
      const int w = px1[r] - px0[r] + 1, nfrag = w * (py1[r] - py0[r] + 1);
      for (int f = (int)sub; f < nfrag; f += SPLAT_LANES) {
        const int fy = f / w, px = px0[r] + (f - fy * w), py = py0[r] + fy;
        float z;
        if (!sprite_fragment(cam, S[r], px, py, z)) continue;
        if (z != z) continue;
        const int ly = py - by0;
        if (ly < th) atomicMin(&tile[ly * bw + (px - bx0)], zkey(z, id));
        else atomicMin(&zbuf[px * cam.rows + py], zkey(z, id));
      }
    }
    __syncthreads();
    for (int i = threadIdx.x; i < tn; i += BLK) {
      const unsigned long long k = tile[i];
      if (k != ~0ull) {
        const int ly = i / bw, lx = i - ly * bw;
        atomicMin(&zbuf[(bx0 + lx) * cam.rows + (by0 + ly)], k);
      }
    }
    __syncthreads();
  }
#endif
}

__device__ __forceinline__ f3 fill_vertex_at(const uint16_t* __restrict__ d, const Cam& cam, int sx, int sy, int x, int y, float inv_fx,
                                             float inv_fy) {
  const float z = (float)d[clampi(sy, 0, cam.rows - 1) * cam.cols + clampi(sx, 0, cam.cols - 1)] / 1000.0f;
  return {((float)x - cam.cx) * z * inv_fx, ((float)y - cam.cy) * z * inv_fy, z};
}
__device__ __forceinline__ void fill_in_px(const Cam& cam, int x, int y, uchar4 si, float4 sv, float4 sn,
                                           const uint16_t* __restrict__ depth_filtered, const uint8_t* __restrict__ rgb3, bool passthrough,
                                           bool passthroughImage, FillMaps out) {
  const int pi = y * cam.cols + x;
  const float inv_fx = 1.0f / cam.fx, inv_fy = 1.0f / cam.fy;
  if (sv.z == 0 || passthrough) {
    const f3 v = fill_vertex_at(depth_filtered, cam, x, y, x, y, inv_fx, inv_fy);
    out.vertex[pi] = make_float4(v.x, v.y, v.z, 1.f);
  } else {
    out.vertex[pi] = sv;
  }
  if (sn.z == 0 || passthrough) {
    const f3 v = fill_vertex_at(depth_filtered, cam, x, y, x, y, inv_fx, inv_fy);
    const f3 vx = fill_vertex_at(depth_filtered, cam, x + 1, y, x + 1, y, inv_fx, inv_fy);
    const f3 vy = fill_vertex_at(depth_filtered, cam, x, y + 1, x, y + 1, inv_fx, inv_fy);
    const f3 nn = normalized(cross(vx - v, vy - v));
    out.normal[pi] = make_float4(nn.x, nn.y, nn.z, 1.f);
  } else {
    out.normal[pi] = sn;
  }
  if ((si.x == 0 && si.y == 0 && si.z == 0) || passthroughImage) {
    out.image[pi] = make_uchar4(rgb3[(size_t)pi * 3], rgb3[(size_t)pi * 3 + 1], rgb3[(size_t)pi * 3 + 2], 255);
  } else {
    out.image[pi] = si;
  }
}
__device__ __forceinline__ void dense_sample(const Cam& cam, int x, int y, uchar4 si, unsigned* counter) {
  if (counter && x % 20 == 10 && y % 20 == 10 && x / 20 < cam.cols / 20 && y / 20 < cam.rows / 20)
    if (si.x > 0 && si.y > 0 && si.z > 0) atomicAdd(counter, 1u);
}

template <bool FUSE_FILL>
__global__ void __launch_bounds__(BLK) k_surface_resolve(const Cam cam, const float* __restrict__ T16, SurfelSoA map, float maxDepth,
                                                          float confThreshold, int time, int maxTime, int timeDelta,
                                                          unsigned long long* zbuf, PredictMaps out, FillMaps fill,
                                                          const uint16_t* __restrict__ depth_filtered, const uint8_t* __restrict__ rgb3,
                                                          bool passthroughImage, unsigned* dense_counter, unsigned* nonempty_flag,
                                                          unsigned nonempty_value) {
  const int lane = threadIdx.x & 63, wave = threadIdx.x >> 6;
  const int px = blockIdx.x * 16 + (wave & 1) * 8 + (lane >> 3), py = blockIdx.y * 16 + (wave >> 1) * 8 + (lane & 7);
  if (px >= cam.cols || py >= cam.rows) return;
  const int pi = py * cam.cols + px, zi = px * cam.rows + py;
  const unsigned long long key = zbuf[zi];
  uchar4 im = make_uchar4(0, 0, 0, 0);
  float4 vt = make_float4(0, 0, 0, 0), nm = make_float4(0, 0, 0, 0);
  uint16_t tm = 0;
  if (key != ZBUF_EMPTY) {
    if (nonempty_flag) *nonempty_flag = nonempty_value;
    zbuf[zi] = ZBUF_EMPTY;
    const uint32_t id = (uint32_t)key;
    const rt34 T = rt34_load16(T16);
    const float4 pc = map.pos_conf[id], ct = map.col_time[id], nr = map.nrm_rad[id];
    const Sprite S = make_sprite(cam, T, pc, ct, nr, maxDepth, confThreshold, (float)time, (float)maxTime, (float)timeDelta);
    float z = 0.f;
    sprite_fragment(cam, S, px, py, z);
    const f3 col = decodeColor(ct.x);
    im = make_uchar4((uint8_t)roundf(col.x * 255.0f), (uint8_t)roundf(col.y * 255.0f), (uint8_t)roundf(col.z * 255.0f), 255);
    const float fcx = (float)px + 0.5f, fcy = (float)py + 0.5f;
    vt = make_float4((fcx - cam.cx) * z * (1.f / cam.fx), (fcy - cam.cy) * z * (1.f / cam.fy), z, pc.w);
    nm = make_float4(S.n.x, S.n.y, S.n.z, nr.w);
    tm = (uint16_t)(unsigned)ct.z;
  }
  out.image[pi] = im;
  out.vertex[pi] = vt;
  out.normal[pi] = nm;
  out.time[pi] = tm;
  if (FUSE_FILL) {
    fill_in_px(cam, px, py, im, vt, nm, depth_filtered, rgb3, false, passthroughImage, fill);
    dense_sample(cam, px, py, im, dense_counter);
  }
}
__device__ __forceinline__ float depth_of_key(uint32_t k) { return __uint_as_float((k & 0x80000000u) ? (k & 0x7fffffffu) : ~k); }
__global__ void __launch_bounds__(BLK) k_depth_resolve(int cols, int rows, unsigned long long* zbuf, float* __restrict__ depth) {
  const int pi = blockIdx.x * blockDim.x + threadIdx.x;
  if (pi >= cols * rows) return;
  const int py = pi / cols, px = pi - py * cols, zi = px * rows + py;
  const unsigned long long key = zbuf[zi];
  float z = 0.f;
  if (key != ZBUF_EMPTY) {
    zbuf[zi] = ZBUF_EMPTY;
    z = depth_of_key((uint32_t)(key >> 32));
  }
  depth[pi] = z;
}
__global__ void __launch_bounds__(BLK) k_fill_in(const Cam cam, PredictMaps pred, const uint16_t* __restrict__ depth_filtered,
                                                  const uint8_t* __restrict__ rgb3, bool passthrough, bool passthroughImage, FillMaps out) {
  const int pi = blockIdx.x * blockDim.x + threadIdx.x;
  if (pi >= cam.cols * cam.rows) return;
  const int py = pi / cam.cols, px = pi - py * cam.cols;
  fill_in_px(cam, px, py, pred.image[pi], pred.vertex[pi], pred.normal[pi], depth_filtered, rgb3, passthrough, passthroughImage, out);
}
__global__ void k_dense_count(const Cam cam, const uchar4* __restrict__ image, unsigned* counter) {
  const int dc = cam.cols / 20, dr = cam.rows / 20;
  const int i = blockIdx.x * blockDim.x + threadIdx.x;
  if (i >= dc * dr) return;
  const int b = i / dc, a = i - b * dc;
  const uchar4 t = image[(20 * b + 10) * cam.cols + (20 * a + 10)];
  if (t.x > 0 && t.y > 0 && t.z > 0) atomicAdd(counter, 1u);
}

struct FuseArgs {
  Cam cam;
  const float* pose16;
  int time;
  const uint8_t* rgb3;
  const float* dm;
  const float* dmf;
  IndexMaps im;
  float maxDepth;
  const float* weighting;
};
__global__ void __launch_bounds__(BLK) k_associate(const FuseArgs A, Candidates cand, uint32_t* winner, int colwalk) {
  const Cam cam = A.cam;
  const int qc = cam.cols / 2, qr = cam.rows / 2;
  const int q = (int)(xcd_block() * blockDim.x + threadIdx.x);
  if (q >= qc * qr) return;
  const int qy = colwalk ? q % qr : q / qc, qx = colwalk ? q / qr : q - (q / qc) * qc;
  const int par = A.time % 2;
  const int i = 2 * qx + par, j = 2 * qy + par;
  const int r = qx * qr + qy;
  float4 c_col = make_float4(0, 0, 0, 0);
  if (i < cam.cols && j < cam.rows) {
    const float cx = cam.cx, cy = cam.cy;
    const float inv_fx = (float)(1.0 / (double)cam.fx), inv_fy = (float)(1.0 / (double)cam.fy);
    const DepthF DR{A.dm, cam.cols, cam.rows}, DF{A.dmf, cam.cols, cam.rows};
    const float x = pix_coord(i, cam.cols), y = pix_coord(j, cam.rows);
    const float ftime = (float)A.time;
    const f3 vPosLocal = getVertexF(DR, i, j, x, y, cx, cy, inv_fx, inv_fy);
    const bool sel = ((int)x % 2 == (int)ftime % 2 && (int)y % 2 == (int)ftime % 2);
    const bool nb = !(DR.at(i - 1, j) == 0 || DR.at(i, j - 1) == 0 || DR.at(i + 1, j) == 0 || DR.at(i, j + 1) == 0);
#ifndef EF_ASSOC_LATE_LOADS
    const float zf_c = DF.at(i, j), zf_xf = DF.at(i + 1, j), zf_xb = DF.at(i - 1, j), zf_yf = DF.at(i, j + 1), zf_yb = DF.at(i, j - 1);
    const uint8_t* c = A.rgb3 + (size_t)(j * cam.cols + i) * 3;
    const uint8_t c0 = c[0], c1 = c[1], c2 = c[2];
    const float weighting = *A.weighting;
    uint32_t idx9[3][3];
    float4 vc9[3][3], nr9[3][3];
#pragma unroll
    for (int a = 0; a < 3; ++a) {
      const int tx = clampi(i + a - 1, 0, cam.cols - 1);
#pragma unroll
      for (int b = 0; b < 3; ++b) {
        const int ty = clampi(j + b - 1, 0, cam.rows - 1);
        const int ti = im_texel(A.im, cam, tx, ty);
        idx9[a][b] = A.im.index[ti];
        vc9[a][b] = A.im.vert_conf[ti];
        nr9[a][b] = A.im.norm_rad[ti];
      }
    }
    const rt34 pose = rt34_load16(A.pose16);
#endif
    if (sel && nb && vPosLocal.z > 0 && vPosLocal.z <= A.maxDepth) {
#ifdef EF_ASSOC_LATE_LOADS
      const rt34 pose = rt34_load16(A.pose16);
#endif
      const f3 vPos = xform(pose, vPosLocal);
#ifndef EF_ASSOC_LATE_LOADS
      auto vtx = [&](float z, float xx, float yy) { return f3{(xx - cx) * z * inv_fx, (yy - cy) * z * inv_fy, z}; };
      const f3 vPosition_f = vtx(zf_c, x, y);
      const f3 col{(float)c0 / 255.0f, (float)c1 / 255.0f, (float)c2 / 255.0f};
      const f3 xf = vtx(zf_xf, x + 1, y), xb = vtx(zf_xb, x - 1, y), yf = vtx(zf_yf, x, y + 1), yb = vtx(zf_yb, x, y - 1);
      const f3 del_x = half_sum(xb, vPosition_f) - half_sum(xf, vPosition_f);
      const f3 del_y = half_sum(yb, vPosition_f) - half_sum(yf, vPosition_f);
      const f3 vNormLocal = normalized(cross(del_x, del_y));
#else
      const f3 vPosition_f = getVertexF(DF, i, j, x, y, cx, cy, inv_fx, inv_fy);
      const uint8_t* c = A.rgb3 + (size_t)(j * cam.cols + i) * 3;
      const f3 col{(float)c[0] / 255.0f, (float)c[1] / 255.0f, (float)c[2] / 255.0f};
      const f3 vNormLocal = getNormalF(DF, vPosition_f, i, j, x, y, cx, cy, inv_fx, inv_fy);
      const float weighting = *A.weighting;
#endif
      const f3 nW = mul(pose.R, vNormLocal);
      int counter = 0;
      uint32_t best = 0;
      float bestDist = 1000;
      const float xl = (x - cx) * inv_fx, yl = (y - cy) * inv_fy;
      const float lambda = sqrtf(xl * xl + yl * yl + 1);
      const f3 ray{xl, yl, 1};
      const float lenRay = sqrtf(dot(ray, ray));
      const float lenN = sqrtf(dot(vNormLocal, vNormLocal));
#ifdef EF_ASSOC_LATE_LOADS
      uint32_t idx9[3][3];
      float4 vc9[3][3], nr9[3][3];
#pragma unroll
      for (int a = 0; a < 3; ++a) {
        const int tx = clampi(i + a - 1, 0, cam.cols - 1);
#pragma unroll
        for (int b = 0; b < 3; ++b) {
          const int ty = clampi(j + b - 1, 0, cam.rows - 1);
          const int ti = im_texel(A.im, cam, tx, ty);
          idx9[a][b] = A.im.index[ti];
          vc9[a][b] = A.im.vert_conf[ti];
          nr9[a][b] = A.im.norm_rad[ti];
        }
      }
#endif
#pragma unroll
      for (int a = 0; a < 4; ++a) {
        const int a3 = a == 0 ? 0 : (a == 3 ? 2 : 1);
#pragma unroll
        for (int b = 0; b < 4; ++b) {
          const int b3 = b == 0 ? 0 : (b == 3 ? 2 : 1);
          const uint32_t current = idx9[a3][b3];
          if (current > 0U) {
            const float4 vc = vc9[a3][b3];
            if (fabsf((vc.z * lambda) - (vPosLocal.z * lambda)) < 0.05f) {
              const f3 cr = cross(ray, f3{vc.x, vc.y, vc.z});
              const float dist = sqrtf(dot(cr, cr)) / lenRay;
              const float4 nr = nr9[a3][b3];
              const f3 nn{nr.x, nr.y, nr.z};
              const float cang = dot(nn, vNormLocal) / (sqrtf(dot(nn, nn)) * lenN);
              const bool angOk = (cang > 0.87758255f && cang <= 1.0f);
              if (dist < bestDist && (fabsf(nr.z) < 0.75f || angOk)) {
                counter++;
                bestDist = dist;
                best = current;
              }
            }
          }
        }
      }
      const float tag = counter > 0 ? -1.0f : -2.0f;
      cand.pos_conf[r] = make_float4(vPos.x, vPos.y, vPos.z, confidence(x, y, cx, cy, weighting));
      cand.nrm_rad[r] = make_float4(nW.x, nW.y, nW.z, getRadius(vPosition_f.z, vNormLocal.z, inv_fx, inv_fy));
      c_col = make_float4(encodeColor(col), 0.f, ftime, tag);
      cand.best[r] = best;
      if (counter > 0) atomicMin(&winner[best], (uint32_t)r);
    }
  }
  cand.col_time[r] = c_col;
}
__device__ __forceinline__ void merge_surfel(const Candidates& cand, int r, uint32_t id, const SurfelSoA& map, int time, float4& s, float4& sc) {
  const float4 ucol = cand.col_time[r];
  const float4 u = cand.pos_conf[r], un = cand.nrm_rad[r];
  float4 sn = map.nrm_rad[id];
  const float c_k = s.w, a = u.w, ftime = (float)time;
  if (un.w < (1.0f + 0.5f) * sn.w) {
    s.x = ((c_k * s.x) + (a * u.x)) / (c_k + a);
    s.y = ((c_k * s.y) + (a * u.y)) / (c_k + a);
    s.z = ((c_k * s.z) + (a * u.z)) / (c_k + a);
    s.w = c_k + a;
    const f3 oldCol = decodeColor(sc.x), newCol = decodeColor(ucol.x);
    const f3 avg{((c_k * oldCol.x) + (a * newCol.x)) / (c_k + a), ((c_k * oldCol.y) + (a * newCol.y)) / (c_k + a),
                 ((c_k * oldCol.z) + (a * newCol.z)) / (c_k + a)};
    sc.x = encodeColor(avg);
    sc.w = ftime;
    const float nx = ((c_k * sn.x) + (a * un.x)) / (c_k + a), ny = ((c_k * sn.y) + (a * un.y)) / (c_k + a),
                nz = ((c_k * sn.z) + (a * un.z)) / (c_k + a), nw = ((c_k * sn.w) + (a * un.w)) / (c_k + a);
    const f3 nn = normalized(f3{nx, ny, nz});
    sn = make_float4(nn.x, nn.y, nn.z, nw);
    map.pos_conf[id] = s;
    map.col_time[id] = sc;
    map.nrm_rad[id] = sn;
  } else {
    s.w = c_k + a;
    sc.w = ftime;
    map.pos_conf[id] = s;
    map.col_time[id] = sc;
  }
}
__global__ void __launch_bounds__(BLK) k_merge(Candidates cand, const uint32_t* __restrict__ winner, SurfelSoA map, int time) {
  const int r = blockIdx.x * blockDim.x + threadIdx.x;
  if (r >= cand.n) return;
  if (cand.col_time[r].w != -1.0f) return;
  const uint32_t id = cand.best[r];
  if (winner[id] != (uint32_t)r) return;
  float4 s = map.pos_conf[id], sc = map.col_time[id];
  merge_surfel(cand, r, id, map, time, s, sc);
}

struct CleanArgs {
  Cam cam;
  const float* T16;
  int time;
  IndexMaps im;
  float confThreshold;
  int timeDelta;
};
struct Taps3 { int u[3]; int m[3]; };
__device__ __forceinline__ Taps3 dedupe_taps(float x, int hi) {
  int t[4];
#pragma unroll
  for (int a = 0; a < 4; ++a) t[a] = clampi((int)floorf(x + (-1.0f + 0.5f * a)), 0, hi);
  Taps3 r;
  r.u[0] = t[0];
  r.u[2] = t[3];
  r.u[1] = (t[1] != t[0] && t[1] != t[3]) ? t[1] : t[2];
  r.m[0] = 1 + (t[1] == t[0]) + (t[2] == t[0]) + (t[3] == t[0]);
  r.m[2] = (t[3] != t[0]) ? (1 + (t[0] == t[3]) + (t[1] == t[3]) + (t[2] == t[3])) : 0;
  r.m[1] = (r.u[1] != t[0] && r.u[1] != t[3]) ? ((t[1] == r.u[1]) + (t[2] == r.u[1])) : 0;
  return r;
}
__device__ __forceinline__ bool clean_test(const CleanArgs& A, const rt34& T, float4 pc, float4 ct, float4 nr) {
  const Cam& cam = A.cam;
  const float ftime = (float)A.time, ftd = (float)A.timeDelta;
  int test = 1;
  const f3 localPos = xform(T, f3{pc.x, pc.y, pc.z});
  const float x = ((cam.fx * localPos.x) / localPos.z) + cam.cx;
  const float y = ((cam.fy * localPos.y) / localPos.z) + cam.cy;
  const f3 localNorm = normalized(mul(T.R, f3{nr.x, nr.y, nr.z}));
  int cnt = 0, zCount = 0;
  const float tagTime = ct.w == -2 ? ftime : ct.w;
#ifdef EF_CLEAN_ALL_TAPS
  const bool decided = false;
  (void)tagTime;
#else
  const bool decided = tagTime == -1 || ((ftime - tagTime) > 20 && pc.w < A.confThreshold);
#endif
  if (!decided && ftime - ct.w < ftd && localPos.z > 0 && x > 0 && y > 0 && x < (float)cam.cols && y < (float)cam.rows) {
    const Taps3 tx = dedupe_taps(x, cam.cols - 1), ty = dedupe_taps(y, cam.rows - 1);
    uint32_t idx[9];
    float4 vcs[9], c2s[9];
#pragma unroll
    for (int a = 0; a < 3; ++a)
#pragma unroll
      for (int b = 0; b < 3; ++b) {
        const int ti = im_texel(A.im, cam, tx.u[a], ty.u[b]);
        idx[a * 3 + b] = A.im.index[ti];
        vcs[a * 3 + b] = A.im.vert_conf[ti];
        c2s[a * 3 + b] = A.im.color_time[ti];
      }
    const bool steep = fabsf(localNorm.z) > 0.85f;
#pragma unroll
    for (int a = 0; a < 3; ++a)
#pragma unroll
      for (int b = 0; b < 3; ++b) {
        const int w = tx.m[a] * ty.m[b];
        const float4 vc = vcs[a * 3 + b], c2 = c2s[a * 3 + b];
        if (w > 0 && idx[a * 3 + b] > 0U) {
          const float dx = vc.x - localPos.x, dy = vc.y - localPos.y;
          if (c2.z < ct.z && vc.w > A.confThreshold && vc.z > localPos.z && vc.z - localPos.z < 0.01f &&
              sqrtf(dx * dx + dy * dy) < nr.w * 1.4f)
            cnt += w;
          if (c2.w == ftime && vc.w > A.confThreshold && vc.z > localPos.z && vc.z - localPos.z > 0.01f && steep)
            zCount += w;
        }
      }
  }
  if (cnt > 8 || zCount > 4) test = 0;
  float lastTime = ct.w;
  if (lastTime == -2) lastTime = ftime;
  if (lastTime == -1 || ((ftime - lastTime) > 20 && pc.w < A.confThreshold)) test = 0;
  if (lastTime > 0 && ftime - lastTime > ftd) test = 1;
  return test != 0;
}
__device__ __forceinline__ bool load_element(const SurfelSoA& map, const Candidates& cand, unsigned count, unsigned e, float4& pc,
                                             float4& ct, float4& nr) {
  if (e < count) {
    pc = map.pos_conf[e]; ct = map.col_time[e]; nr = map.nrm_rad[e];
    return true;
  }
  const unsigned r = e - count;
  ct = cand.col_time[r];
  if (ct.w == 0.0f) return false;
  pc = cand.pos_conf[r]; nr = cand.nrm_rad[r];
  return true;
}
struct DeformArgs {
  const float* graph;
  int nodes;
  const float* depth;
  int isFern;
  float maxDepth;
};
__device__ __forceinline__ float node_tex(const DeformArgs& D, int idx) {
  idx = clampi(idx, 0, 16384 - 1);
  return idx < D.nodes * 16 ? D.graph[idx] : 0.0f;
}
__device__ __forceinline__ f3 node_pos(const DeformArgs& D, int j) { return f3{node_tex(D, j * 16), node_tex(D, j * 16 + 1), node_tex(D, j * 16 + 2)}; }
__device__ __forceinline__ float node_dist(const DeformArgs& D, f3 pos, int j) {
  const f3 d = pos - node_pos(D, j);
  return sqrtf(dot(d, d));
}
struct M3c { float m[3][3]; };
__device__ __forceinline__ f3 mulc(const M3c& a, f3 v) {
  return {dot(f3{a.m[0][0], a.m[1][0], a.m[2][0]}, v), dot(f3{a.m[0][1], a.m[1][1], a.m[2][1]}, v), dot(f3{a.m[0][2], a.m[1][2], a.m[2][2]}, v)};
}
__device__ __forceinline__ M3c inverse3(const M3c& a) {
  const float (*m)[3] = a.m;
  const float c00 = m[1][1] * m[2][2] - m[2][1] * m[1][2], c01 = m[2][1] * m[0][2] - m[0][1] * m[2][2], c02 = m[0][1] * m[1][2] - m[1][1] * m[0][2];
  const float det = (m[0][0] * c00 + m[1][0] * c01) + m[2][0] * c02;
  const float id = 1.0f / det;
  M3c r;
  r.m[0][0] = c00 * id; r.m[0][1] = c01 * id; r.m[0][2] = c02 * id;
  r.m[1][0] = (m[2][0] * m[1][2] - m[1][0] * m[2][2]) * id; r.m[1][1] = (m[0][0] * m[2][2] - m[2][0] * m[0][2]) * id; r.m[1][2] = (m[1][0] * m[0][2] - m[0][0] * m[1][2]) * id;
  r.m[2][0] = (m[1][0] * m[2][1] - m[2][0] * m[1][1]) * id; r.m[2][1] = (m[2][0] * m[0][1] - m[0][0] * m[2][1]) * id; r.m[2][2] = (m[0][0] * m[1][1] - m[1][0] * m[0][1]) * id;
  return r;
}
__device__ void deform_vertex(const CleanArgs& A, const DeformArgs& D, const rt34& T, float4& pc, float4& ct, float4& nr) {
  constexpr int k = 4, lookBack = 20;
  const int nodes = D.nodes;
  int nearNodes[lookBack];
  float nearDists[lookBack];
  for (int i = 0; i < lookBack; ++i) { nearNodes[i] = -1; nearDists[i] = 16777216.0f; }
  const int poseTime = (int)ct.z;
  int foundIndex = 0, imin = 0, imax = nodes - 1, imid = (imin + imax) / 2;
  while (imax >= imin) {
    imid = (imin + imax) / 2;
    const int nodeTime = (int)node_tex(D, imid * 16 + 15);
    if (nodeTime < poseTime) imin = imid + 1;
    else if (nodeTime > poseTime) imax = imid - 1;
    else break;
  }
  imin = min(imin, nodes - 1);
  const int nodeMin = (int)node_tex(D, imin * 16 + 15), nodeMid = (int)node_tex(D, imid * 16 + 15), nodeMax = (int)node_tex(D, imax * 16 + 15);
  if (abs(nodeMin - poseTime) <= abs(nodeMid - poseTime) && abs(nodeMin - poseTime) <= abs(nodeMax - poseTime)) foundIndex = imin;
  else if (abs(nodeMid - poseTime) <= abs(nodeMin - poseTime) && abs(nodeMid - poseTime) <= abs(nodeMax - poseTime)) foundIndex = imid;
  else foundIndex = imax;
  if (foundIndex == nodes) foundIndex = nodes - 1;
  const f3 pos{pc.x, pc.y, pc.z};
  int nearNodeIndex = 0, distanceBack = 0;
  for (int j = foundIndex; j >= 0; --j) {
    nearNodes[nearNodeIndex] = j;
    nearDists[nearNodeIndex] = node_dist(D, pos, j);
    nearNodeIndex++;
    if (++distanceBack == lookBack / 2) break;
  }
  for (int j = foundIndex + 1; j < nodes; ++j) {
    nearNodes[nearNodeIndex] = j;
    nearDists[nearNodeIndex] = node_dist(D, pos, j);
    nearNodeIndex++;
    if (++distanceBack == lookBack) break;
  }
  for (int i = 0; i < lookBack - 1; ++i)
    for (int j = i + 1; j < lookBack; ++j)
      if (nearDists[j] < nearDists[i]) {
        const float tf = nearDists[i]; nearDists[i] = nearDists[j]; nearDists[j] = tf;
        const int ti = nearNodes[i]; nearNodes[i] = nearNodes[j]; nearNodes[j] = ti;
      }
  const float dMax = nearDists[k];
  float nodeWeights[k];
  float weightSum = 0;
  for (int j = 0; j < k; ++j) {
    const float q = 1.0f - (node_dist(D, pos, nearNodes[j]) / dMax);
    nodeWeights[j] = q * q;
    weightSum += nodeWeights[j];
  }
  for (int j = 0; j < k; ++j) nodeWeights[j] /= weightSum;
  f3 newPos{0.f, 0.f, 0.f}, newNorm{0.f, 0.f, 0.f};
  const f3 nrm{nr.x, nr.y, nr.z};
  for (int i = 0; i < k; ++i) {
    const int n = nearNodes[i];
    const f3 g = node_pos(D, n);
    M3c R;
    for (int c = 0; c < 3; ++c)
      for (int r = 0; r < 3; ++r) R.m[c][r] = node_tex(D, n * 16 + 3 + c * 3 + r);
    const f3 t{node_tex(D, n * 16 + 12), node_tex(D, n * 16 + 13), node_tex(D, n * 16 + 14)};
    const f3 moved = (mulc(R, pos - g) + g) + t;
    newPos = newPos + f3{nodeWeights[i] * moved.x, nodeWeights[i] * moved.y, nodeWeights[i] * moved.z};
    const M3c Ri = inverse3(R);
    M3c Rit;
    for (int c = 0; c < 3; ++c)
      for (int r = 0; r < 3; ++r) Rit.m[c][r] = Ri.m[r][c];
    const f3 rn = mulc(Rit, nrm);
    newNorm = newNorm + f3{nodeWeights[i] * rn.x, nodeWeights[i] * rn.y, nodeWeights[i] * rn.z};
  }
  pc.x = newPos.x; pc.y = newPos.y; pc.z = newPos.z;
  const f3 nn = normalized(newNorm);
  nr.x = nn.x; nr.y = nn.y; nr.z = nn.z;
  if (pc.w > A.confThreshold && D.isFern == 0) {
    const Cam& cam = A.cam;
    const f3 lp = xform(T, f3{pc.x, pc.y, pc.z});
    const float x = ((cam.fx * lp.x) / lp.z) + cam.cx, y = ((cam.fy * lp.y) / lp.z) + cam.cy;
    if (lp.z > 0 && lp.z < D.maxDepth && x > 0 && y > 0 && x < (float)cam.cols && y < (float)cam.rows) {
      const float currentDepth = D.depth[clampi((int)floorf(y), 0, cam.rows - 1) * cam.cols + clampi((int)floorf(x), 0, cam.cols - 1)];
      if (currentDepth > 0.0f && lp.z < currentDepth + 0.1f) ct.w = (float)A.time;
    }
  }
}
__global__ void __launch_bounds__(BLK) k_clean_deform(const CleanArgs A, const DeformArgs D, SurfelSoA map, const unsigned* __restrict__ count_dev,
                                                       Candidates cand, const uint8_t* __restrict__ flags) {
  const unsigned count = *count_dev;
  const unsigned n = count + (unsigned)cand.n;
  const rt34 T = rt34_load16(A.T16);
  for (unsigned e = blockIdx.x * blockDim.x + threadIdx.x; e < n; e += gridDim.x * blockDim.x) {
    if (!flags[e]) continue;
    float4* ppc = e < count ? &map.pos_conf[e] : &cand.pos_conf[e - count];
    float4* pct = e < count ? &map.col_time[e] : &cand.col_time[e - count];
    float4* pnr = e < count ? &map.nrm_rad[e] : &cand.nrm_rad[e - count];
    float4 pc = *ppc, ct = *pct, nr = *pnr;
    if (ct.w == -2.0f) ct.w = (float)A.time;
    if (ct.z == (float)A.time) { *pct = ct; continue; }
    deform_vertex(A, D, T, pc, ct, nr);
    *ppc = pc; *pct = ct; *pnr = nr;
  }
}

__global__ void __launch_bounds__(BLK) k_clean_flags(const CleanArgs A, SurfelSoA map, const unsigned* __restrict__ count_dev,
                                                      Candidates cand, uint32_t* winner, uint8_t* __restrict__ flags,
                                                      uint32_t* __restrict__ chunk_count, uint32_t* gsum_now, uint32_t* __restrict__ gsum_zero,
                                                      int max_groups) {
  __shared__ unsigned lds[BLK / 64];
  const unsigned count = *count_dev;
  const unsigned n = count + (unsigned)cand.n;
  const unsigned nrows = (n + CLEAN_ROW - 1) / CLEAN_ROW;
  const rt34 T = rt34_load16(A.T16);
  if (gsum_zero)
    for (int i = blockIdx.x * BLK + threadIdx.x; i < max_groups; i += gridDim.x * BLK) gsum_zero[(size_t)i * CLEAN_GSTRIDE] = 0u;
  unsigned r;
  for (unsigned it = 0; xcd_row(nrows, it, r); ++it) {
    const unsigned e = r * CLEAN_ROW + threadIdx.x;
    bool f = false;
    if (e < n) {
      float4 pc, ct, nr;
      if (load_element(map, cand, count, e, pc, ct, nr)) f = clean_test(A, T, pc, ct, nr);
      if (e < count) winner[e] = WINNER_EMPTY;
      flags[e] = f ? 1 : 0;
    }
    const unsigned wave_keep = (unsigned)__popcll(__ballot(f));
    if ((threadIdx.x & 63) == 0) lds[threadIdx.x >> 6] = wave_keep;
    __syncthreads();
    if (threadIdx.x == 0) {
      unsigned tot = 0;
#pragma unroll
      for (int i = 0; i < BLK / 64; ++i) tot += lds[i];
      chunk_count[r] = tot;
      if (gsum_now && tot) atomicAdd(&gsum_now[(size_t)(r / CLEAN_GROUP) * CLEAN_GSTRIDE], tot);
    }
    __syncthreads();
  }
}
__device__ __forceinline__ unsigned block_excl_scan_and_sum(unsigned v, unsigned a, unsigned* lds, unsigned& total, unsigned& asum) {
  const int t = threadIdx.x, lane = t & 63, w = t >> 6;
  unsigned x = v, y = a;
#pragma unroll
  for (int off = 1; off < 64; off <<= 1) {
    const unsigned u = __shfl_up(x, off, 64);
    if (lane >= off) x += u;
    y += __shfl_xor(y, off, 64);
  }
  __syncthreads();
  if (lane == 63) { lds[w] = x; lds[BLK / 64 + w] = y; }
  __syncthreads();
  unsigned base = 0, tot = 0, as = 0;
#pragma unroll
  for (int i = 0; i < BLK / 64; ++i) {
    const unsigned s = lds[i];
    if (i < w) base += s;
    tot += s;
    as += lds[BLK / 64 + i];
  }
  total = tot;
  asum = as;
  return base + x - v;
}
__global__ void __launch_bounds__(BLK) k_clean_scatter(SurfelSoA map, const unsigned* __restrict__ count_dev, Candidates cand,
                                                        const uint8_t* __restrict__ flags, const uint32_t* __restrict__ chunk_offset,
                                                        int time, SurfelSoA out, uint32_t capacity, const uint32_t* __restrict__ gsum,
                                                        const uint32_t* __restrict__ chunk_count, uint32_t* total_out, unsigned* count_out,
                                                        int* overflow_flag) {
  __shared__ unsigned lds[2 * BLK / 64];
  const unsigned count = *count_dev;
  const unsigned n = count + (unsigned)cand.n;
  const unsigned nrows = (n + CLEAN_ROW - 1) / CLEAN_ROW;
  if (gsum && nrows == 0 && blockIdx.x == 0 && threadIdx.x == 0) {
    *total_out = 0u;
    if (count_out) *count_out = 0u;
  }
  unsigned r;
  for (unsigned it = 0; xcd_row(nrows, it, r); ++it) {
    const unsigned e = r * CLEAN_ROW + threadIdx.x;
    const unsigned f = (e < n) ? flags[e] : 0u;
    unsigned before = 0;
    if (gsum) {
      const unsigned g = r / CLEAN_GROUP;
      for (unsigned i = threadIdx.x; i < g; i += BLK) before += gsum[(size_t)i * CLEAN_GSTRIDE];
      for (unsigned i = g * CLEAN_GROUP + threadIdx.x; i < r; i += BLK) before += chunk_count[i];
    }
    float4 pc = make_float4(0, 0, 0, 0), ct = pc, nr = pc;
    if (f) load_element(map, cand, count, e, pc, ct, nr);
    unsigned tot, row0;
    unsigned pos = block_excl_scan_and_sum(f, before, lds, tot, row0);
    if (!gsum) row0 = chunk_offset[r];
    pos += row0;
    if (f && pos < capacity) {
      if (ct.w == -2.0f) ct.w = (float)time;
      out.pos_conf[pos] = pc;
      out.col_time[pos] = ct;
      out.nrm_rad[pos] = nr;
    }
    if (gsum && r == nrows - 1 && threadIdx.x == 0) {
      unsigned all = row0 + tot;
      *total_out = all;
      if (count_out) {
        if (all > capacity) { all = capacity; if (overflow_flag) *overflow_flag = 1; }
        *count_out = all;
      }
    }
    __syncthreads();
  }
}

__global__ void __launch_bounds__(BLK) k_cand_flags(Candidates cand, uint8_t* __restrict__ flags, uint32_t* __restrict__ chunk_count) {
  __shared__ unsigned lds[BLK / 64];
  const unsigned n = cand.n, c = blockIdx.x;
  unsigned keep = 0;
  for (int k = 0; k < 4; ++k) {
    const unsigned e = c * CHUNK + k * BLK + threadIdx.x;
    if (e < n) {
      const uint8_t f = cand.col_time[e].w != 0.0f;
      flags[e] = f;
      keep += f;
    }
  }
  unsigned tot;
  block_excl_scan(keep, lds, tot);
  if (threadIdx.x == 0) chunk_count[c] = tot;
}
__global__ void __launch_bounds__(BLK) k_cand_scatter(Candidates cand, const uint8_t* __restrict__ flags,
                                                       const uint32_t* __restrict__ chunk_offset, float4* __restrict__ aos) {
  __shared__ unsigned lds[BLK / 64];
  const unsigned n = cand.n, c = blockIdx.x;
  unsigned base = chunk_offset[c];
  for (int k = 0; k < 4; ++k) {
    const unsigned e = c * CHUNK + k * BLK + threadIdx.x;
    const unsigned f = (e < n) ? flags[e] : 0u;
    unsigned tot;
    const unsigned pos = base + block_excl_scan(f, lds, tot);
    if (f) {
      aos[(size_t)pos * 3] = cand.pos_conf[e];
      aos[(size_t)pos * 3 + 1] = cand.col_time[e];
      aos[(size_t)pos * 3 + 2] = cand.nrm_rad[e];
    }
    base += tot;
    __syncthreads();
  }
}

}

static inline dim3 tgrid(int cols, int rows) { return dim3(ceil_div(cols, 64), ceil_div(rows, 4)); }

const float* bilateral_table() {
  static std::mutex mu;
  static float* tables[64] = {};
  int dev = 0;
  if (hipGetDevice(&dev) != hipSuccess || dev < 0 || dev >= 64) return nullptr;
  std::lock_guard<std::mutex> lk(mu);
  if (!tables[dev]) {
    float* p = nullptr;
    if (hipMalloc(&p, sizeof(float) * BIL_ROWS * BIL_COLS) != hipSuccess) return nullptr;
    hipLaunchKernelGGL(k_bilateral_table, dim3(ceil_div(BIL_ROWS * BIL_COLS, 256)), dim3(256), 0, (hipStream_t)0, p);
    if (hipDeviceSynchronize() != hipSuccess) { (void)hipFree(p); return nullptr; }
    tables[dev] = p;
  }
  return tables[dev];
}
bool filter_depth(const uint16_t* raw, int cols, int rows, float maxD, uint16_t* filtered, hipStream_t s) {
  const float* table = bilateral_table();
  if (!table) return false;
  hipLaunchKernelGGL(k_preprocess<false>, dim3(ceil_div(cols, PRE_TW), ceil_div(rows, PRE_TH)), dim3(64, 4), 0, s, raw, cols, rows, (unsigned)(maxD * 1000.0f), table,
                     filtered, (float*)nullptr, (float*)nullptr, (const uint8_t*)nullptr, (uint8_t*)nullptr, (uint8_t*)nullptr);
  return true;
}
void metricise_depth(const uint16_t* in, int cols, int rows, float maxD, float* out, hipStream_t s) {
  hipLaunchKernelGGL(k_metricise, dim3(ceil_div(cols * rows, 256)), dim3(256), 0, s, in, cols * rows, (unsigned)(maxD * 1000.0f), out);
}
bool preprocess_depth(const uint16_t* raw, int cols, int rows, float maxD, uint16_t* filtered, float* metric, float* metric_filtered,
                      hipStream_t s, unsigned extra_lds, const uint8_t* rgb3, uint8_t* next0, uint8_t* rgb_keep, const float* table) {
  if (!table) table = bilateral_table();
  if (!table) return false;
  constexpr unsigned STATIC_LDS = sizeof(float) * (BIL_ROWS * BIL_COLS + PRE_LH * PRE_LW);
  static_assert(STATIC_LDS < 65536u, "k_preprocess fits the default LDS limit");
  if (extra_lds > 65536u - STATIC_LDS) extra_lds = 65536u - STATIC_LDS;
  hipLaunchKernelGGL(k_preprocess<true>, dim3(ceil_div(cols, PRE_TW), ceil_div(rows, PRE_TH)), dim3(64, 4), extra_lds, s, raw, cols, rows, (unsigned)(maxD * 1000.0f), table,
                     filtered, metric, metric_filtered, rgb3, next0, rgb_keep);
  return true;
}
namespace {
__global__ void k_copy_map(SurfelSoA src, const unsigned* __restrict__ count_dev, SurfelSoA dst) {
  const unsigned n = *count_dev;
  for (unsigned i = blockIdx.x * blockDim.x + threadIdx.x; i < n; i += gridDim.x * blockDim.x) {
    dst.pos_conf[i] = src.pos_conf[i];
    dst.col_time[i] = src.col_time[i];
    dst.nrm_rad[i] = src.nrm_rad[i];
  }
}
}
void copy_map(SurfelSoA src, const unsigned* count_dev, SurfelSoA dst, hipStream_t s) {
  hipLaunchKernelGGL(k_copy_map, dim3(SURFEL_GRID), dim3(BLK), 0, s, src, count_dev, dst);
}
void aos_to_soa(const float* aos, uint32_t count, SurfelSoA soa, hipStream_t s) {
  if (count) hipLaunchKernelGGL(k_aos_to_soa, dim3(ceil_div((int)count, 256)), dim3(256), 0, s, (const float4*)aos, count, soa);
}
void soa_to_aos(SurfelSoA soa, uint32_t count, float* aos, hipStream_t s) {
  if (count) hipLaunchKernelGGL(k_soa_to_aos, dim3(ceil_div((int)count, 256)), dim3(256), 0, s, soa, count, (float4*)aos);
}

void seed_map(const Cam& cam, const uint8_t* rgb3, const float* dm, const float* dmf, int time, float maxDepth, SurfelSoA out,
              unsigned* count_dev, const CompactScratch& cs, hipStream_t s) {
  const int P = cam.cols * cam.rows;
  const int nch = ceil_div(P, CHUNK);
  SeedArgs A{cam, rgb3, dm, dmf, time, maxDepth};
  uint8_t* fr = cs.flags;
  uint8_t* ff = cs.flags + P;
  uint32_t* cr = cs.chunk_count;
  uint32_t* cf = cs.chunk_count + nch;
  uint32_t* orw = cs.chunk_offset;
  uint32_t* ofl = cs.chunk_offset + nch;
  (void)hipMemsetAsync(out.nrm_rad, 0, (size_t)P * sizeof(float4), s);
  hipLaunchKernelGGL(k_seed_flags, dim3(nch), dim3(BLK), 0, s, A, fr, ff, cr, cf);
  hipLaunchKernelGGL(k_scan_chunks, dim3(1), dim3(1024), 0, s, (const uint32_t*)cr, (const unsigned*)nullptr, (unsigned)P, orw, cs.totals);
  hipLaunchKernelGGL(k_scan_chunks, dim3(1), dim3(1024), 0, s, (const uint32_t*)cf, (const unsigned*)nullptr, (unsigned)P, ofl, cs.totals + 1);
  hipLaunchKernelGGL(k_seed_scatter, dim3(nch), dim3(BLK), 0, s, A, (const uint8_t*)fr, (const uint8_t*)ff, (const uint32_t*)orw,
                     (const uint32_t*)ofl, (const uint32_t*)cs.totals, out, count_dev);
}

void predict_indices(const Cam& cam, const float* T_cw16_dev, int time, SurfelSoA map, const unsigned* count_dev, float maxDepth,
                     int timeDelta, unsigned long long* zbuf, IndexMaps out, hipStream_t s, eft::KernelProbe* probe, const Candidates* merge_cand,
                     const uint32_t* merge_winner) {
  if (merge_cand) {
    hipLaunchKernelGGL(k_index_splat<true>, dim3(SURFEL_GRID), dim3(BLK), 0, s, cam, T_cw16_dev, time, map, count_dev, maxDepth, timeDelta, zbuf,
                       out.colmajor, *merge_cand, merge_winner);
    hipLaunchKernelGGL(k_index_resolve, dim3(ceil_div(cam.cols * cam.rows, BLK)), dim3(BLK), 0, s, cam, T_cw16_dev, map, zbuf, out);
    return;
  }
  const bool sample = probe && probe->used < probe->capacity;
  hipEvent_t e0 = sample ? probe->start[probe->used] : nullptr, e1 = sample ? probe->stop[probe->used] : nullptr;
  if (sample) probe->used++;
  hipExtLaunchKernelGGL(k_index_splat<false>, dim3(SURFEL_GRID), dim3(BLK), 0, s, e0, e1, 0, cam, T_cw16_dev, time, map, count_dev, maxDepth, timeDelta,
                        zbuf, out.colmajor, Candidates{}, (const uint32_t*)nullptr);
  hipLaunchKernelGGL(k_index_resolve, dim3(ceil_div(cam.cols * cam.rows, BLK)), dim3(BLK), 0, s, cam, T_cw16_dev, map, zbuf, out);
}

void combined_predict(const Cam& cam, const float* T_cw16_dev, SurfelSoA map, const unsigned* count_dev, float maxDepth,
                      float confThreshold, int time, int maxTime, int timeDelta, unsigned long long* zbuf, PredictMaps out, FillMaps fill,
                      const uint16_t* depth_filtered, const uint8_t* rgb3, bool passthroughImage, unsigned* dense_counter, hipStream_t s,
                      unsigned* nonempty_flag, unsigned nonempty_value, unsigned* consumed_mark, unsigned consumed_value, const float* rays4) {
#ifdef EF_SPLAT_NO_LUT
  rays4 = nullptr;
#endif
  if (rays4)
    hipLaunchKernelGGL(k_surface_splat<true>, dim3(SPLAT_GRID), dim3(BLK), 0, s, cam, T_cw16_dev, map, count_dev, maxDepth, confThreshold,
                       time, maxTime, timeDelta, zbuf, consumed_mark, consumed_value, (const float4*)rays4);
  else
    hipLaunchKernelGGL(k_surface_splat<false>, dim3(SPLAT_GRID), dim3(BLK), 0, s, cam, T_cw16_dev, map, count_dev, maxDepth, confThreshold,
                       time, maxTime, timeDelta, zbuf, consumed_mark, consumed_value, (const float4*)nullptr);
  const dim3 g(ceil_div(cam.cols, 16), ceil_div(cam.rows, 16));
  if (fill.image)
    hipLaunchKernelGGL(k_surface_resolve<true>, g, dim3(BLK), 0, s, cam, T_cw16_dev, map, maxDepth, confThreshold, time, maxTime, timeDelta,
                       zbuf, out, fill, depth_filtered, rgb3, passthroughImage, dense_counter, nonempty_flag, nonempty_value);
  else
    hipLaunchKernelGGL(k_surface_resolve<false>, g, dim3(BLK), 0, s, cam, T_cw16_dev, map, maxDepth, confThreshold, time, maxTime, timeDelta,
                       zbuf, out, fill, depth_filtered, rgb3, passthroughImage, dense_counter, nonempty_flag, nonempty_value);
}
void synthesize_depth(const Cam& cam, const float* T_cw16_dev, SurfelSoA map, const unsigned* count_dev, float maxDepth, float confThreshold,
                      int time, int maxTime, int timeDelta, unsigned long long* zbuf, float* depth, hipStream_t s, const float* rays4) {
  if (rays4)
    hipLaunchKernelGGL(k_surface_splat<true>, dim3(SPLAT_GRID), dim3(BLK), 0, s, cam, T_cw16_dev, map, count_dev, maxDepth, confThreshold,
                       time, maxTime, timeDelta, zbuf, (unsigned*)nullptr, 0u, (const float4*)rays4);
  else
    hipLaunchKernelGGL(k_surface_splat<false>, dim3(SPLAT_GRID), dim3(BLK), 0, s, cam, T_cw16_dev, map, count_dev, maxDepth, confThreshold,
                       time, maxTime, timeDelta, zbuf, (unsigned*)nullptr, 0u, (const float4*)nullptr);
  const int n = cam.cols * cam.rows;
  hipLaunchKernelGGL(k_depth_resolve, dim3(ceil_div(n, BLK)), dim3(BLK), 0, s, cam.cols, cam.rows, zbuf, depth);
}
void build_ray_table(const Cam& cam, float* rays4, hipStream_t s) {
  hipLaunchKernelGGL(k_ray_table, dim3(ceil_div(cam.cols * cam.rows, BLK)), dim3(BLK), 0, s, cam, (float4*)rays4);
}
void fill_in(const Cam& cam, PredictMaps pred, const uint16_t* depth_filtered, const uint8_t* rgb3, bool passthrough, bool passthroughImage,
             FillMaps out, hipStream_t s) {
  hipLaunchKernelGGL(k_fill_in, dim3(ceil_div(cam.cols * cam.rows, BLK)), dim3(BLK), 0, s, cam, pred, depth_filtered, rgb3, passthrough,
                     passthroughImage, out);
}
void dense_count(const Cam& cam, const uchar4* image, unsigned* counter, hipStream_t s) {
  const int n = (cam.cols / 20) * (cam.rows / 20);
  hipLaunchKernelGGL(k_dense_count, dim3(ceil_div(n, 256)), dim3(256), 0, s, cam, image, counter);
}

void fuse(const Cam& cam, const float* pose_f16_dev, int time, const uint8_t* rgb3, const float* dm, const float* dmf, IndexMaps im,
          float maxDepth, const float* weighting_dev, SurfelSoA map, const unsigned* count_dev, Candidates cand, uint32_t* winner,
          hipStream_t s, bool defer_merge) {
  (void)count_dev;
  FuseArgs A{cam, pose_f16_dev, time, rgb3, dm, dmf, im, maxDepth, weighting_dev};
  hipLaunchKernelGGL(k_associate, dim3(ceil_div(cand.n, BLK)), dim3(BLK), 0, s, A, cand, winner, im.colmajor ? 1 : 0);
  if (!defer_merge) hipLaunchKernelGGL(k_merge, dim3(ceil_div(cand.n, BLK)), dim3(BLK), 0, s, cand, (const uint32_t*)winner, map, time);
}

void clean(const Cam& cam, const float* T_cw16_dev, int time, IndexMaps im, float confThreshold, int timeDelta, SurfelSoA map,
           const unsigned* count_dev, Candidates cand, uint32_t* winner, SurfelSoA out, unsigned* count_out_dev, uint32_t capacity,
           const CompactScratch& cs, int* overflow_flag, hipStream_t s, const Deformation* deform) {
  CleanArgs A{cam, T_cw16_dev, time, im, confThreshold, timeDelta};
#ifdef EF_SEPARATE_SCAN
  const bool fold = false;
#else
  const bool fold = cs.group_sum != nullptr;
#endif
  uint32_t* const gnow = fold ? cs.group_sum + (size_t)(cs.flip & 1) * cs.max_groups * CLEAN_GSTRIDE : nullptr;
  uint32_t* const gzero = fold ? cs.group_sum + (size_t)((cs.flip & 1) ^ 1) * cs.max_groups * CLEAN_GSTRIDE : nullptr;
  hipLaunchKernelGGL(k_clean_flags, dim3(CLEAN_GRID), dim3(BLK), 0, s, A, map, count_dev, cand, winner, cs.flags,
                     cs.chunk_count, gnow, gzero, cs.max_groups);
  if (deform && deform->nodes > 0) {
    const DeformArgs D{deform->graph_dev, deform->nodes, deform->depth_dev, deform->is_fern, deform->max_depth};
    hipLaunchKernelGGL(k_clean_deform, dim3(CLEAN_GRID), dim3(BLK), 0, s, A, D, map, count_dev, cand, (const uint8_t*)cs.flags);
  }
  if (!fold)
    hipLaunchKernelGGL(k_scan_chunks, dim3(1), dim3(1024), 0, s, (const uint32_t*)cs.chunk_count, (const unsigned*)count_dev, (unsigned)cand.n,
                       cs.chunk_offset, cs.totals, count_out_dev, capacity, overflow_flag, (unsigned)CLEAN_ROW);
  hipLaunchKernelGGL(k_clean_scatter, dim3(CLEAN_GRID), dim3(BLK), 0, s, map, count_dev, cand, (const uint8_t*)cs.flags,
                     (const uint32_t*)cs.chunk_offset, time, out, capacity, (const uint32_t*)gnow, (const uint32_t*)cs.chunk_count, cs.totals,
                     count_out_dev, overflow_flag);
}

void candidates_to_aos(Candidates cand, float* aos, unsigned* count_dev, const CompactScratch& cs, hipStream_t s) {
  const int nch = ceil_div(cand.n, CHUNK);
  hipLaunchKernelGGL(k_cand_flags, dim3(nch), dim3(BLK), 0, s, cand, cs.flags, cs.chunk_count);
  hipLaunchKernelGGL(k_scan_chunks, dim3(1), dim3(1024), 0, s, (const uint32_t*)cs.chunk_count, (const unsigned*)nullptr, (unsigned)cand.n,
                     cs.chunk_offset, count_dev);
  hipLaunchKernelGGL(k_cand_scatter, dim3(nch), dim3(BLK), 0, s, cand, (const uint8_t*)cs.flags, (const uint32_t*)cs.chunk_offset, (float4*)aos);
}

__global__ void k_sample_graph(SurfelSoA map, const unsigned* __restrict__ count_dev, int stride, int max_nodes, float4* __restrict__ out,
                               unsigned* __restrict__ n_out) {
  const int i = blockIdx.x * blockDim.x + threadIdx.x;
  const unsigned count = *count_dev;
  const unsigned n = count == 0 ? 0u : (count - 1u) / (unsigned)stride + 1u;
  if (i == 0) *n_out = n < (unsigned)max_nodes ? n : (unsigned)max_nodes;
  if (i >= max_nodes || (unsigned)i >= n) return;
  const float4 p = map.pos_conf[(size_t)i * stride];
  const float4 c = map.col_time[(size_t)i * stride];
  out[i] = make_float4(p.x, p.y, p.z, c.z);
}
void sample_graph(SurfelSoA map, const unsigned* count_dev, int stride, int max_nodes, float* out4, unsigned* n_out, hipStream_t s) {
  hipLaunchKernelGGL(k_sample_graph, dim3(ceil_div(max_nodes, 256)), dim3(256), 0, s, map, count_dev, stride, max_nodes, (float4*)out4, n_out);
}

#include "ef_render.inc"
#include "ef_labels.inc"
#include "ef_query.inc"
#include "ef_register.inc"

}
```

Measured before the change: 2063.

## Skip index-map resolve passes; read z-buffer keys directly in associate and clean

In the default fast path, the two per-frame index-map resolve kernels are no longer launched. The associate and clean kernels instead read 64-bit depth/id keys from dedicated z-buffers, filter taps by depth decoded from the key, and gather surfel attributes from the map, transforming them on the fly. Clearing of the alternate z-buffers is folded into the associate and scatter kernels. Resolved maps are materialised lazily only when a host image request needs them. This removes two full-frame write passes and their reads, at the cost of more random gathers from the surfel map and extra arithmetic per tap.

```diff
diff --git a/elasticfusion_amd/build.py b/elasticfusion_amd/build.py
--- a/elasticfusion_amd/build.py
+++ b/elasticfusion_amd/build.py
@@ -48,6 +48,7 @@
     "pipepoll": ["-DEF_FT_PIPELINED_POLL"],
     "pipepoll_clocks": ["-DEF_FT_PIPELINED_POLL", "-DEF_STAGE_CLOCKS"],
     "alltaps": ["-DEF_CLEAN_ALL_TAPS"],
+    "resolve": ["-DEF_KEEP_INDEX_RESOLVE"],
     "r6m": ["-DEF_SEPARATE_SCAN", "-DEF_END_ONE_WAVE"],
 }
 SHIM_LIB = os.path.join(HERE, "libefusion.so")
diff --git a/elasticfusion_amd/csrc/ef_context.hip b/elasticfusion_amd/csrc/ef_context.hip
--- a/elasticfusion_amd/csrc/ef_context.hip
+++ b/elasticfusion_amd/csrc/ef_context.hip
@@ -71,6 +71,11 @@
   efm::PredictMaps pm{};
   efm::FillMaps fm{};
   unsigned long long* zbuf = nullptr;
+  unsigned long long* zbuf_assoc = nullptr;
+  unsigned long long* zbuf_clean = nullptr;
+  float* im_T16 = nullptr;
+  bool im_pending = false;
+  int im_map = 0;
   efm::SurfelSoA maps[2]{};
   int cur = 0;
   efm::SurfelSoA shadow{};
@@ -836,8 +841,14 @@
 #ifndef EF_RESOLVE_ALL_MAPS
       im_assoc.color_time = nullptr;
 #endif
-      efm::predict_indices(c->cam, c->st->T_cw, c->tick, c->maps[c->cur], &c->st->map_counts[c->cur], c->maxDepthProcessed, c->cfg.time_delta, c->zbuf,
-                           im_assoc, s, sample_splat ? &c->probe_splat : nullptr);
+#ifdef EF_KEEP_INDEX_RESOLVE
+      const bool keyed = false;
+#else
+      const bool keyed = !c->timing && !c->reference_download && !c->cfg.close_loops;
+#endif
+      const efm::KeyedIndex key_assoc{c->zbuf_assoc, c->st->T_cw, c->maps[c->cur]}, key_clean{c->zbuf_clean, c->st->T_cw, c->maps[c->cur]};
+      efm::predict_indices(c->cam, c->st->T_cw, c->tick, c->maps[c->cur], &c->st->map_counts[c->cur], c->maxDepthProcessed, c->cfg.time_delta,
+                           keyed ? c->zbuf_assoc : c->zbuf, im_assoc, s, sample_splat ? &c->probe_splat : nullptr, nullptr, nullptr, !keyed);
       timer_end(c, "indexMap");
       timer_begin(c, "Fuse::Data+Update");
 #ifdef EF_SEPARATE_MERGE
@@ -846,12 +857,15 @@
       const bool defer_merge = !c->timing;
 #endif
       efm::fuse(c->cam, c->st->pose_f, c->tick, c->rgb, c->depth_metric, c->depth_metric_filtered, c->im, c->maxDepthProcessed,
-                &c->st->weighting, c->maps[c->cur], &c->st->map_counts[c->cur], c->cand, c->winner, s, defer_merge);
+                &c->st->weighting, c->maps[c->cur], &c->st->map_counts[c->cur], c->cand, c->winner, s, defer_merge,
+                keyed ? &key_assoc : nullptr, keyed ? c->zbuf_clean : nullptr);
       if (c->reference_download && !defer_merge) efm::copy_map(c->maps[c->cur], &c->st->map_counts[c->cur], c->shadow, s);
       timer_end(c, "Fuse::Data+Update");
       timer_begin(c, "indexMap2");
-      efm::predict_indices(c->cam, c->st->T_cw, c->tick, c->maps[c->cur], &c->st->map_counts[c->cur], c->maxDepthProcessed, c->cfg.time_delta, c->zbuf,
-                           c->im, s, nullptr, defer_merge ? &c->cand : nullptr, c->winner);
+      efm::predict_indices(c->cam, c->st->T_cw, c->tick, c->maps[c->cur], &c->st->map_counts[c->cur], c->maxDepthProcessed, c->cfg.time_delta,
+                           keyed ? c->zbuf_clean : c->zbuf, c->im, s, nullptr, defer_merge ? &c->cand : nullptr, c->winner, !keyed);
+      c->im_pending = keyed;
+      c->im_map = c->cur;
       if (c->reference_download && defer_merge) efm::copy_map(c->maps[c->cur], &c->st->map_counts[c->cur], c->shadow, s);
       timer_end(c, "indexMap2");
       efm::Deformation def{c->graph_dev, c->graph_nodes, c->synth_depth, c->graph_is_fern, c->maxDepthProcessed};
@@ -862,7 +876,7 @@
       c->cs.flip ^= 1;
       efm::clean(c->cam, c->st->T_cw, c->tick, c->im, c->cfg.confidence, c->cfg.time_delta, c->maps[c->cur], &c->st->map_counts[c->cur], c->cand,
                  c->winner, c->maps[c->cur ^ 1], &c->st->map_counts[c->cur ^ 1], c->capacity, c->cs, c->overflow, s,
-                 c->graph_nodes > 0 ? &def : nullptr);
+                 c->graph_nodes > 0 ? &def : nullptr, keyed ? &key_clean : nullptr, keyed ? c->zbuf_assoc : nullptr, keyed ? c->im_T16 : nullptr);
       c->graph_nodes = 0;
       c->cur ^= 1;
       timer_end(c, "Fuse::Copy");
@@ -955,6 +969,9 @@
   EF_ALLOC(c, c->fm.vertex, P);
   EF_ALLOC(c, c->fm.normal, P);
   EF_ALLOC(c, c->zbuf, P, 0xFF);
+  EF_ALLOC(c, c->zbuf_assoc, P, 0xFF);
+  EF_ALLOC(c, c->zbuf_clean, P, 0xFF);
+  EF_ALLOC(c, c->im_T16, 16);
   EF_ALLOC(c, c->graph_dev, 1024 * 16);
   EF_ALLOC(c, c->synth_depth, P);
   EF_ALLOC(c, c->rays, P * 4);
@@ -1738,10 +1755,16 @@
 int ef_set_confidence_threshold(ef_ctx* c, float v) { if (!c) return EF_EINVAL; c->cfg.confidence = v; return EF_OK; }
 int ef_set_depth_cutoff(ef_ctx* c, float v) { if (!c) return EF_EINVAL; c->cfg.depth_cut = v; return EF_OK; }
 
+static void im_materialise(ef_ctx* c) {
+  if (!c->im_pending) return;
+  efm::resolve_indices(c->cam, c->im_T16, c->maps[c->im_map], c->zbuf_clean, c->im, c->stream);
+  c->im_pending = false;
+}
 int ef_get_image(ef_ctx* c, int which, void* dst, size_t bytes) {
   if (!c || !dst) return EF_EINVAL;
   DeviceGuard dg_(c);
   const size_t P = (size_t)c->cam.cols * c->cam.rows;
+  if (which >= EF_IMG_INDEX && which <= EF_IMG_NORM_RAD) im_materialise(c);
   const void* src = nullptr;
   size_t need = 0;
   switch (which) {
diff --git a/elasticfusion_amd/csrc/ef_map.hpp b/elasticfusion_amd/csrc/ef_map.hpp
--- a/elasticfusion_amd/csrc/ef_map.hpp
+++ b/elasticfusion_amd/csrc/ef_map.hpp
@@ -28,6 +28,11 @@
 __host__ __device__ inline int im_texel(const IndexMaps& im, const Cam& cam, int px, int py) {
   return im.colmajor ? px * cam.rows + py : py * cam.cols + px;
 }
+struct KeyedIndex {
+  const unsigned long long* keys;
+  const float* T_cw16_dev;
+  SurfelSoA map;
+};
 struct PredictMaps {
   uchar4* image;
   float4* vertex;
@@ -75,7 +80,9 @@
 
 void predict_indices(const Cam& cam, const float* T_cw16_dev, int time, SurfelSoA map, const unsigned* count_dev, float maxDepth,
                      int timeDelta, unsigned long long* zbuf, IndexMaps out, hipStream_t s, eft::KernelProbe* probe = nullptr,
-                     const struct Candidates* merge_cand = nullptr, const uint32_t* merge_winner = nullptr);
+                     const struct Candidates* merge_cand = nullptr, const uint32_t* merge_winner = nullptr,
+                     bool resolve = true);
+void resolve_indices(const Cam& cam, const float* T_cw16_dev, SurfelSoA map, const unsigned long long* zbuf, IndexMaps out, hipStream_t s);
 void combined_predict(const Cam& cam, const float* T_cw16_dev, SurfelSoA map, const unsigned* count_dev, float maxDepth,
                       float confThreshold, int time, int maxTime, int timeDelta, unsigned long long* zbuf, PredictMaps out,
                       FillMaps fill, const uint16_t* depth_filtered, const uint8_t* rgb3, bool passthroughImage,
@@ -93,7 +100,8 @@
 
 void fuse(const Cam& cam, const float* pose_f16_dev, int time, const uint8_t* rgb3, const float* depth_metric,
           const float* depth_metric_filtered, IndexMaps im, float maxDepth, const float* weighting_dev, SurfelSoA map,
-          const unsigned* count_dev, Candidates cand, uint32_t* winner, hipStream_t s, bool defer_merge = false);
+          const unsigned* count_dev, Candidates cand, uint32_t* winner, hipStream_t s, bool defer_merge = false,
+          const KeyedIndex* keyed = nullptr, unsigned long long* zclear = nullptr);
 struct Deformation {
   const float* graph_dev;
   int nodes;
@@ -103,7 +111,8 @@
 };
 void clean(const Cam& cam, const float* T_cw16_dev, int time, IndexMaps im, float confThreshold, int timeDelta, SurfelSoA map,
            const unsigned* count_dev, Candidates cand, uint32_t* winner, SurfelSoA out, unsigned* count_out_dev, uint32_t capacity,
-           const CompactScratch& cs, int* overflow_flag, hipStream_t s, const Deformation* deform = nullptr);
+           const CompactScratch& cs, int* overflow_flag, hipStream_t s, const Deformation* deform = nullptr,
+           const KeyedIndex* keyed = nullptr, unsigned long long* zclear = nullptr, float* T_keep16_dev = nullptr);
 void sample_graph(SurfelSoA map, const unsigned* count_dev, int stride, int max_nodes, float* out4, unsigned* n_out, hipStream_t s);
 void candidates_to_aos(Candidates cand, float* aos, unsigned* count_dev, const CompactScratch& cs, hipStream_t s);
 
diff --git a/elasticfusion_amd/csrc/ef_map_kernels.hip b/elasticfusion_amd/csrc/ef_map_kernels.hip
--- a/elasticfusion_amd/csrc/ef_map_kernels.hip
+++ b/elasticfusion_amd/csrc/ef_map_kernels.hip
@@ -3,6 +3,7 @@
 #include <mutex>
 #include <hip/hip_ext.h>
 #include "ef_map.hpp"
+#include "ef_zkey.hpp"
 
 using namespace ef;
 
@@ -17,10 +18,6 @@
 static_assert(CLEAN_ROW == BLK, "clean kernels run one element per thread");
 static_assert(CLEAN_GRID % 8 == 0, "xcd_row");
 
-__device__ __forceinline__ uint32_t depth_key(float z) {
-  const uint32_t b = __float_as_uint(z);
-  return (b & 0x80000000u) ? ~b : (b | 0x80000000u);
-}
 __device__ __forceinline__ unsigned long long zkey(float z, uint32_t id) { return ((unsigned long long)depth_key(z) << 32) | id; }
 __device__ __forceinline__ unsigned xcd_block() {
   const unsigned g = gridDim.x, x = blockIdx.x & 7u, slot = blockIdx.x >> 3;
@@ -310,6 +307,15 @@
     atomicMin(&zbuf[colmajor ? px * cam.rows + py : py * cam.cols + px], zkey(p.z, id));
   }
 }
+__device__ __forceinline__ float4 index_texel_vert_conf(const rt34& T, float4 pc) {
+  const f3 p = xform(T, f3{pc.x, pc.y, pc.z});
+  return make_float4(p.x, p.y, p.z, pc.w);
+}
+__device__ __forceinline__ float4 index_texel_norm_rad(const rt34& T, float4 nr) {
+  const f3 n = normalized(mul(T.R, f3{nr.x, nr.y, nr.z}));
+  return make_float4(n.x, n.y, n.z, nr.w);
+}
+template <bool CLEAR>
 __global__ void __launch_bounds__(BLK) k_index_resolve(const Cam cam, const float* __restrict__ T16, SurfelSoA map,
                                                         unsigned long long* zbuf, IndexMaps out) {
   const int pi = blockIdx.x * blockDim.x + threadIdx.x;
@@ -322,17 +328,15 @@
     out.norm_rad[pi] = make_float4(0, 0, 0, 0);
     return;
   }
-  zbuf[pi] = ZBUF_EMPTY;
+  if (CLEAR) zbuf[pi] = ZBUF_EMPTY;
   const uint32_t id = (uint32_t)key;
   const rt34 T = rt34_load16(T16);
   const float4 pc = map.pos_conf[id];
   const float4 nr = map.nrm_rad[id];
-  const f3 p = xform(T, f3{pc.x, pc.y, pc.z});
-  const f3 n = normalized(mul(T.R, f3{nr.x, nr.y, nr.z}));
   out.index[pi] = id;
-  out.vert_conf[pi] = make_float4(p.x, p.y, p.z, pc.w);
+  out.vert_conf[pi] = index_texel_vert_conf(T, pc);
   if (out.color_time) out.color_time[pi] = map.col_time[id];
-  out.norm_rad[pi] = make_float4(n.x, n.y, n.z, nr.w);
+  out.norm_rad[pi] = index_texel_norm_rad(T, nr);
 }
 
 struct Sprite {
@@ -596,7 +600,6 @@
     dense_sample(cam, px, py, im, dense_counter);
   }
 }
-__device__ __forceinline__ float depth_of_key(uint32_t k) { return __uint_as_float((k & 0x80000000u) ? (k & 0x7fffffffu) : ~k); }
 __global__ void __launch_bounds__(BLK) k_depth_resolve(int cols, int rows, unsigned long long* zbuf, float* __restrict__ depth) {
   const int pi = blockIdx.x * blockDim.x + threadIdx.x;
   if (pi >= cols * rows) return;
@@ -635,11 +638,16 @@
   IndexMaps im;
   float maxDepth;
   const float* weighting;
+  KeyedIndex key;
+  unsigned long long* zclear;
 };
+template <bool KEYED>
 __global__ void __launch_bounds__(BLK) k_associate(const FuseArgs A, Candidates cand, uint32_t* winner, int colwalk) {
   const Cam cam = A.cam;
   const int qc = cam.cols / 2, qr = cam.rows / 2;
   const int q = (int)(xcd_block() * blockDim.x + threadIdx.x);
+  if (KEYED && A.zclear)
+    for (int i = q, P = cam.cols * cam.rows, step = (int)(gridDim.x * blockDim.x); i < P; i += step) A.zclear[i] = ZBUF_EMPTY;
   if (q >= qc * qr) return;
   const int qy = colwalk ? q % qr : q / qc, qx = colwalk ? q / qr : q - (q / qc) * qc;
   const int par = A.time % 2;
@@ -662,6 +670,7 @@
     const float weighting = *A.weighting;
     uint32_t idx9[3][3];
     float4 vc9[3][3], nr9[3][3];
+    uint2 key9[3][3];
 #pragma unroll
     for (int a = 0; a < 3; ++a) {
       const int tx = clampi(i + a - 1, 0, cam.cols - 1);
@@ -669,9 +678,13 @@
       for (int b = 0; b < 3; ++b) {
         const int ty = clampi(j + b - 1, 0, cam.rows - 1);
         const int ti = im_texel(A.im, cam, tx, ty);
-        idx9[a][b] = A.im.index[ti];
-        vc9[a][b] = A.im.vert_conf[ti];
-        nr9[a][b] = A.im.norm_rad[ti];
+        if (KEYED) {
+          key9[a][b] = reinterpret_cast<const uint2*>(A.key.keys)[ti];
+        } else {
+          idx9[a][b] = A.im.index[ti];
+          vc9[a][b] = A.im.vert_conf[ti];
+          nr9[a][b] = A.im.norm_rad[ti];
+        }
       }
     }
     const rt34 pose = rt34_load16(A.pose16);
@@ -708,6 +721,7 @@
 #ifdef EF_ASSOC_LATE_LOADS
       uint32_t idx9[3][3];
       float4 vc9[3][3], nr9[3][3];
+      uint2 key9[3][3];
 #pragma unroll
       for (int a = 0; a < 3; ++a) {
         const int tx = clampi(i + a - 1, 0, cam.cols - 1);
@@ -715,12 +729,36 @@
         for (int b = 0; b < 3; ++b) {
           const int ty = clampi(j + b - 1, 0, cam.rows - 1);
           const int ti = im_texel(A.im, cam, tx, ty);
-          idx9[a][b] = A.im.index[ti];
-          vc9[a][b] = A.im.vert_conf[ti];
-          nr9[a][b] = A.im.norm_rad[ti];
+          if (KEYED) {
+            key9[a][b] = reinterpret_cast<const uint2*>(A.key.keys)[ti];
+          } else {
+            idx9[a][b] = A.im.index[ti];
+            vc9[a][b] = A.im.vert_conf[ti];
+            nr9[a][b] = A.im.norm_rad[ti];
+          }
         }
       }
 #endif
+      const rt34 Tcw = rt34_load16(KEYED ? A.key.T_cw16_dev : A.pose16);
+      if (KEYED) {
+#pragma unroll
+        for (int a = 0; a < 3; ++a)
+#pragma unroll
+          for (int b = 0; b < 3; ++b) {
+            const uint32_t id = key9[a][b].x;
+            float vcz = depth_of_key(key9[a][b].y);
+            asm volatile("" : "+v"(vcz));
+            const bool tap = (id & key9[a][b].y) != 0xFFFFFFFFu  && id > 0U && fabsf((vcz * lambda) - (vPosLocal.z * lambda)) < 0.05f;
+            idx9[a][b] = tap ? id : 0U;
+          }
+#pragma unroll
+        for (int a = 0; a < 3; ++a)
+#pragma unroll
+          for (int b = 0; b < 3; ++b) {
+            vc9[a][b] = A.key.map.pos_conf[idx9[a][b]];
+            nr9[a][b] = A.key.map.nrm_rad[idx9[a][b]];
+          }
+      }
 #pragma unroll
       for (int a = 0; a < 4; ++a) {
         const int a3 = a == 0 ? 0 : (a == 3 ? 2 : 1);
@@ -729,11 +767,11 @@
           const int b3 = b == 0 ? 0 : (b == 3 ? 2 : 1);
           const uint32_t current = idx9[a3][b3];
           if (current > 0U) {
-            const float4 vc = vc9[a3][b3];
+            const float4 vc = KEYED ? index_texel_vert_conf(Tcw, vc9[a3][b3]) : vc9[a3][b3];
             if (fabsf((vc.z * lambda) - (vPosLocal.z * lambda)) < 0.05f) {
               const f3 cr = cross(ray, f3{vc.x, vc.y, vc.z});
               const float dist = sqrtf(dot(cr, cr)) / lenRay;
-              const float4 nr = nr9[a3][b3];
+              const float4 nr = KEYED ? index_texel_norm_rad(Tcw, nr9[a3][b3]) : nr9[a3][b3];
               const f3 nn{nr.x, nr.y, nr.z};
               const float cang = dot(nn, vNormLocal) / (sqrtf(dot(nn, nn)) * lenN);
               const bool angOk = (cang > 0.87758255f && cang <= 1.0f);
@@ -802,6 +840,7 @@
   IndexMaps im;
   float confThreshold;
   int timeDelta;
+  KeyedIndex key;
 };
 struct Taps3 { int u[3]; int m[3]; };
 __device__ __forceinline__ Taps3 dedupe_taps(float x, int hi) {
@@ -817,6 +856,7 @@
   r.m[1] = (r.u[1] != t[0] && r.u[1] != t[3]) ? ((t[1] == r.u[1]) + (t[2] == r.u[1])) : 0;
   return r;
 }
+template <bool KEYED>
 __device__ __forceinline__ bool clean_test(const CleanArgs& A, const rt34& T, float4 pc, float4 ct, float4 nr) {
   const Cam& cam = A.cam;
   const float ftime = (float)A.time, ftd = (float)A.timeDelta;
@@ -837,22 +877,44 @@
     const Taps3 tx = dedupe_taps(x, cam.cols - 1), ty = dedupe_taps(y, cam.rows - 1);
     uint32_t idx[9];
     float4 vcs[9], c2s[9];
-#pragma unroll
-    for (int a = 0; a < 3; ++a)
-#pragma unroll
-      for (int b = 0; b < 3; ++b) {
-        const int ti = im_texel(A.im, cam, tx.u[a], ty.u[b]);
-        idx[a * 3 + b] = A.im.index[ti];
-        vcs[a * 3 + b] = A.im.vert_conf[ti];
-        c2s[a * 3 + b] = A.im.color_time[ti];
+    if (KEYED) {
+      unsigned long long keys[9];
+#pragma unroll
+      for (int a = 0; a < 3; ++a)
+#pragma unroll
+        for (int b = 0; b < 3; ++b) keys[a * 3 + b] = A.key.keys[im_texel(A.im, cam, tx.u[a], ty.u[b])];
+#pragma unroll
+      for (int a = 0; a < 3; ++a)
+#pragma unroll
+        for (int b = 0; b < 3; ++b) {
+          const unsigned long long key = keys[a * 3 + b];
+          const uint32_t id = (uint32_t)key;
+          const bool tap = tx.m[a] * ty.m[b] > 0 && key != ZBUF_EMPTY && id > 0U && depth_of_key((uint32_t)(key >> 32)) > localPos.z;
+          idx[a * 3 + b] = tap ? id : 0U;
+        }
+#pragma unroll
+      for (int k = 0; k < 9; ++k) {
+        vcs[k] = A.key.map.pos_conf[idx[k]];
+        c2s[k] = A.key.map.col_time[idx[k]];
       }
+    } else {
+#pragma unroll
+      for (int a = 0; a < 3; ++a)
+#pragma unroll
+        for (int b = 0; b < 3; ++b) {
+          const int ti = im_texel(A.im, cam, tx.u[a], ty.u[b]);
+          idx[a * 3 + b] = A.im.index[ti];
+          vcs[a * 3 + b] = A.im.vert_conf[ti];
+          c2s[a * 3 + b] = A.im.color_time[ti];
+        }
+    }
     const bool steep = fabsf(localNorm.z) > 0.85f;
 #pragma unroll
     for (int a = 0; a < 3; ++a)
 #pragma unroll
       for (int b = 0; b < 3; ++b) {
         const int w = tx.m[a] * ty.m[b];
-        const float4 vc = vcs[a * 3 + b], c2 = c2s[a * 3 + b];
+        const float4 vc = KEYED ? index_texel_vert_conf(T, vcs[a * 3 + b]) : vcs[a * 3 + b], c2 = c2s[a * 3 + b];
         if (w > 0 && idx[a * 3 + b] > 0U) {
           const float dx = vc.x - localPos.x, dy = vc.y - localPos.y;
           if (c2.z < ct.z && vc.w > A.confThreshold && vc.z > localPos.z && vc.z - localPos.z < 0.01f &&
@@ -1012,6 +1074,7 @@
   }
 }
 
+template <bool KEYED>
 __global__ void __launch_bounds__(BLK) k_clean_flags(const CleanArgs A, SurfelSoA map, const unsigned* __restrict__ count_dev,
                                                       Candidates cand, uint32_t* winner, uint8_t* __restrict__ flags,
                                                       uint32_t* __restrict__ chunk_count, uint32_t* gsum_now, uint32_t* __restrict__ gsum_zero,
@@ -1029,7 +1092,7 @@
     bool f = false;
     if (e < n) {
       float4 pc, ct, nr;
-      if (load_element(map, cand, count, e, pc, ct, nr)) f = clean_test(A, T, pc, ct, nr);
+      if (load_element(map, cand, count, e, pc, ct, nr)) f = clean_test<KEYED>(A, T, pc, ct, nr);
       if (e < count) winner[e] = WINNER_EMPTY;
       flags[e] = f ? 1 : 0;
     }
@@ -1074,8 +1137,12 @@
                                                         const uint8_t* __restrict__ flags, const uint32_t* __restrict__ chunk_offset,
                                                         int time, SurfelSoA out, uint32_t capacity, const uint32_t* __restrict__ gsum,
                                                         const uint32_t* __restrict__ chunk_count, uint32_t* total_out, unsigned* count_out,
-                                                        int* overflow_flag) {
+                                                        int* overflow_flag, unsigned long long* __restrict__ zclear, int zclear_n,
+                                                        const float* __restrict__ T_src, float* __restrict__ T_keep) {
   __shared__ unsigned lds[2 * BLK / 64];
+  if (zclear)
+    for (int i = blockIdx.x * BLK + threadIdx.x; i < zclear_n; i += gridDim.x * BLK) zclear[i] = ZBUF_EMPTY;
+  if (T_keep && blockIdx.x == 0 && threadIdx.x < 16) T_keep[threadIdx.x] = T_src[threadIdx.x];
   const unsigned count = *count_dev;
   const unsigned n = count + (unsigned)cand.n;
   const unsigned nrows = (n + CLEAN_ROW - 1) / CLEAN_ROW;
@@ -1234,11 +1301,11 @@
 
 void predict_indices(const Cam& cam, const float* T_cw16_dev, int time, SurfelSoA map, const unsigned* count_dev, float maxDepth,
                      int timeDelta, unsigned long long* zbuf, IndexMaps out, hipStream_t s, eft::KernelProbe* probe, const Candidates* merge_cand,
-                     const uint32_t* merge_winner) {
+                     const uint32_t* merge_winner, bool resolve) {
   if (merge_cand) {
     hipLaunchKernelGGL(k_index_splat<true>, dim3(SURFEL_GRID), dim3(BLK), 0, s, cam, T_cw16_dev, time, map, count_dev, maxDepth, timeDelta, zbuf,
                        out.colmajor, *merge_cand, merge_winner);
-    hipLaunchKernelGGL(k_index_resolve, dim3(ceil_div(cam.cols * cam.rows, BLK)), dim3(BLK), 0, s, cam, T_cw16_dev, map, zbuf, out);
+    if (resolve) hipLaunchKernelGGL(k_index_resolve<true>, dim3(ceil_div(cam.cols * cam.rows, BLK)), dim3(BLK), 0, s, cam, T_cw16_dev, map, zbuf, out);
     return;
   }
   const bool sample = probe && probe->used < probe->capacity;
@@ -1246,7 +1313,11 @@
   if (sample) probe->used++;
   hipExtLaunchKernelGGL(k_index_splat<false>, dim3(SURFEL_GRID), dim3(BLK), 0, s, e0, e1, 0, cam, T_cw16_dev, time, map, count_dev, maxDepth, timeDelta,
                         zbuf, out.colmajor, Candidates{}, (const uint32_t*)nullptr);
-  hipLaunchKernelGGL(k_index_resolve, dim3(ceil_div(cam.cols * cam.rows, BLK)), dim3(BLK), 0, s, cam, T_cw16_dev, map, zbuf, out);
+  if (resolve) hipLaunchKernelGGL(k_index_resolve<true>, dim3(ceil_div(cam.cols * cam.rows, BLK)), dim3(BLK), 0, s, cam, T_cw16_dev, map, zbuf, out);
+}
+void resolve_indices(const Cam& cam, const float* T_cw16_dev, SurfelSoA map, const unsigned long long* zbuf, IndexMaps out, hipStream_t s) {
+  hipLaunchKernelGGL(k_index_resolve<false>, dim3(ceil_div(cam.cols * cam.rows, BLK)), dim3(BLK), 0, s, cam, T_cw16_dev, map,
+                     const_cast<unsigned long long*>(zbuf), out);
 }
 
 void combined_predict(const Cam& cam, const float* T_cw16_dev, SurfelSoA map, const unsigned* count_dev, float maxDepth,
@@ -1296,17 +1367,21 @@
 
 void fuse(const Cam& cam, const float* pose_f16_dev, int time, const uint8_t* rgb3, const float* dm, const float* dmf, IndexMaps im,
           float maxDepth, const float* weighting_dev, SurfelSoA map, const unsigned* count_dev, Candidates cand, uint32_t* winner,
-          hipStream_t s, bool defer_merge) {
+          hipStream_t s, bool defer_merge, const KeyedIndex* keyed, unsigned long long* zclear) {
   (void)count_dev;
-  FuseArgs A{cam, pose_f16_dev, time, rgb3, dm, dmf, im, maxDepth, weighting_dev};
-  hipLaunchKernelGGL(k_associate, dim3(ceil_div(cand.n, BLK)), dim3(BLK), 0, s, A, cand, winner, im.colmajor ? 1 : 0);
+  FuseArgs A{cam, pose_f16_dev, time, rgb3, dm, dmf, im, maxDepth, weighting_dev, keyed ? *keyed : KeyedIndex{}, zclear};
+  if (keyed)
+    hipLaunchKernelGGL(k_associate<true>, dim3(ceil_div(cand.n, BLK)), dim3(BLK), 0, s, A, cand, winner, im.colmajor ? 1 : 0);
+  else
+    hipLaunchKernelGGL(k_associate<false>, dim3(ceil_div(cand.n, BLK)), dim3(BLK), 0, s, A, cand, winner, im.colmajor ? 1 : 0);
   if (!defer_merge) hipLaunchKernelGGL(k_merge, dim3(ceil_div(cand.n, BLK)), dim3(BLK), 0, s, cand, (const uint32_t*)winner, map, time);
 }
 
 void clean(const Cam& cam, const float* T_cw16_dev, int time, IndexMaps im, float confThreshold, int timeDelta, SurfelSoA map,
            const unsigned* count_dev, Candidates cand, uint32_t* winner, SurfelSoA out, unsigned* count_out_dev, uint32_t capacity,
-           const CompactScratch& cs, int* overflow_flag, hipStream_t s, const Deformation* deform) {
-  CleanArgs A{cam, T_cw16_dev, time, im, confThreshold, timeDelta};
+           const CompactScratch& cs, int* overflow_flag, hipStream_t s, const Deformation* deform, const KeyedIndex* keyed,
+           unsigned long long* zclear, float* T_keep16_dev) {
+  CleanArgs A{cam, T_cw16_dev, time, im, confThreshold, timeDelta, keyed ? *keyed : KeyedIndex{}};
 #ifdef EF_SEPARATE_SCAN
   const bool fold = false;
 #else
@@ -1314,8 +1389,12 @@
 #endif
   uint32_t* const gnow = fold ? cs.group_sum + (size_t)(cs.flip & 1) * cs.max_groups * CLEAN_GSTRIDE : nullptr;
   uint32_t* const gzero = fold ? cs.group_sum + (size_t)((cs.flip & 1) ^ 1) * cs.max_groups * CLEAN_GSTRIDE : nullptr;
-  hipLaunchKernelGGL(k_clean_flags, dim3(CLEAN_GRID), dim3(BLK), 0, s, A, map, count_dev, cand, winner, cs.flags,
-                     cs.chunk_count, gnow, gzero, cs.max_groups);
+  if (keyed)
+    hipLaunchKernelGGL(k_clean_flags<true>, dim3(CLEAN_GRID), dim3(BLK), 0, s, A, map, count_dev, cand, winner, cs.flags,
+                       cs.chunk_count, gnow, gzero, cs.max_groups);
+  else
+    hipLaunchKernelGGL(k_clean_flags<false>, dim3(CLEAN_GRID), dim3(BLK), 0, s, A, map, count_dev, cand, winner, cs.flags,
+                       cs.chunk_count, gnow, gzero, cs.max_groups);
   if (deform && deform->nodes > 0) {
     const DeformArgs D{deform->graph_dev, deform->nodes, deform->depth_dev, deform->is_fern, deform->max_depth};
     hipLaunchKernelGGL(k_clean_deform, dim3(CLEAN_GRID), dim3(BLK), 0, s, A, D, map, count_dev, cand, (const uint8_t*)cs.flags);
@@ -1325,7 +1404,7 @@
                        cs.chunk_offset, cs.totals, count_out_dev, capacity, overflow_flag, (unsigned)CLEAN_ROW);
   hipLaunchKernelGGL(k_clean_scatter, dim3(CLEAN_GRID), dim3(BLK), 0, s, map, count_dev, cand, (const uint8_t*)cs.flags,
                      (const uint32_t*)cs.chunk_offset, time, out, capacity, (const uint32_t*)gnow, (const uint32_t*)cs.chunk_count, cs.totals,
-                     count_out_dev, overflow_flag);
+                     count_out_dev, overflow_flag, zclear, cam.cols * cam.rows, T_cw16_dev, T_keep16_dev);
 }
 
 void candidates_to_aos(Candidates cand, float* aos, unsigned* count_dev, const CompactScratch& cs, hipStream_t s) {
diff --git a/elasticfusion_amd/csrc/ef_zkey.hpp b/elasticfusion_amd/csrc/ef_zkey.hpp
--- /dev/null
+++ b/elasticfusion_amd/csrc/ef_zkey.hpp
@@ -0,0 +1,24 @@
+#pragma once
+#include <stdint.h>
+
+#if defined(__HIPCC__)
+#define EF_ZKEY_HD __host__ __device__ __forceinline__
+#else
+#define EF_ZKEY_HD inline
+#endif
+
+namespace efm {
+
+EF_ZKEY_HD uint32_t depth_key(float z) {
+  uint32_t b;
+  __builtin_memcpy(&b, &z, 4);
+  return (b & 0x80000000u) ? ~b : (b | 0x80000000u);
+}
+EF_ZKEY_HD float depth_of_key(uint32_t k) {
+  const uint32_t b = (k & 0x80000000u) ? (k & 0x7fffffffu) : ~k;
+  float z;
+  __builtin_memcpy(&z, &b, 4);
+  return z;
+}
+
+}
```

After: 2130, median of 6. 1.03x the previous value.
